# hku-mars/LiDAR_IMU_Init

Measured on AMD Instinct MI355X. Metric: ICP+ESKF scans/sec @100k pts/scan, higher is better.
Workload: dtype f64; 1 GPU; stream100k: 100000 pts/scan (time-sorted) vs 1000000-pt local map, max_iteration 5, LIO mode (12-col H), static map, voxel-grid leaf 0.05; scans resident in HBM, 8 distinct scans cycled, the state reset to the scan's propagated state every step; map_points=1000000, params=harness/launch/ouster (reference-format yaml + launch), parallelism=points sharded x1, transport=none, rccl_ranks=0

## Files before the change

### lidar_imu_init_amd/csrc/lii_capi.cpp

```cpp
#include "lii_context.h"

using namespace lii_impl;

namespace lii_impl {

thread_local std::string g_err;

static constexpr unsigned kProfEventFlags = hipEventDisableSystemFence;

void harvest_knn_events(lii_handle h) {
  const unsigned int due = h->prof.ev_it_due;
  h->prof.ev_it_due = 0u;
  for (int it = 0; it < 16; it++) {
    if (!((due >> it) & 1u)) continue;
    float kk = 0;
    if (hipEventElapsedTime(&kk, h->prof.ev_it[2 * it], h->prof.ev_it[2 * it + 1]) != hipSuccess) continue;
    h->prof.timings[7] += kk;
    h->prof.timings[5] += 1;
  }
}

int fail(lii_handle h, int code, const std::string& msg) {
  if (h) h->err = msg;
  g_err = msg;
  return code;
}
int kp_mark(lii_handle h, int kind, int it) {
  if (h->prof.prof_mode != 3) return LII_OK;
  if (h->prof.kp_n >= (int)h->prof.kp_ev.size()) {
    lii::Event e;
    if (e.create(kProfEventFlags) != hipSuccess) return fail(h, LII_ERR_HIP, "hipEventCreate (kernel profile)");
    h->prof.kp_ev.push_back(std::move(e));
    h->prof.kp_kind.push_back(0);
  }
  if (hipEventRecord(h->prof.kp_ev[size_t(h->prof.kp_n)], h->stream) != hipSuccess) return fail(h, LII_ERR_HIP, "hipEventRecord (kernel profile)");
  h->prof.kp_kind[size_t(h->prof.kp_n)] = kind * 64 + std::min(it, 63);
  h->prof.kp_n++;
  return LII_OK;
}
GridView grid_view(const lii_context* c) {
  GridView g;
  g.pts = c->d_pts;
  g.blocks = c->d_blocks;
  g.cells = c->d_cells;
  g.block_mask = c->block_mask;
  g.n_pts = c->map_dirty ? std::max(c->n_map, 1) : c->n_map;
  g.cs = c->cell_size;
  g.inv_cs = 1.0f / c->cell_size;
  g.max_d2 = c->cfg.max_match_dist2;
  g.win = (c->win_valid && !c->map_dirty) ? c->d_win : nullptr;
  g.wx0 = c->win_org[0]; g.wy0 = c->win_org[1]; g.wz0 = c->win_org[2];
  g.wnx = c->win_dim[0]; g.wny = c->win_dim[1]; g.wnz = c->win_dim[2];
  return g;
}
RegistrationBuffers reg_buffers(const lii_context* c) {
  RegistrationBuffers rb;
  rb.body = c->d_body;
  rb.world = c->d_world;
  rb.nbr = c->d_nbr;
  rb.nbr_count = c->d_nbr_count;
  rb.plane = c->d_plane;
  rb.selected = c->d_selected;
  rb.partials = c->d_partials;
  rb.partial_stride = c->partial_stride;
  rb.n = c->n_body;
  rb.n_dev = c->n_body_pending ? c->d_nbody : nullptr;
  rb.cap = c->cfg.max_scan_points;
  rb.flag_count = c->d_flags;
  rb.flag_list = reinterpret_cast<float4*>(c->d_flags + 4);
  rb.shard_rank = c->net.rank;
  rb.shard_world = (c->net.n_ranks > 1 && c->net.library_partition && !c->body_partitioned) ? c->net.n_ranks : 1;
  if (c->solo_share < -1 && c->net.n_ranks <= 1) { rb.shard_world = -c->solo_share; rb.shard_rank = 0; }
  return rb;
}
PoseArg pose_of(const lii_state& s) {
  PoseArg p;
  std::memcpy(p.R, s.rot_end, 72);
  std::memcpy(p.p, s.pos_end, 24);
  std::memcpy(p.RLI, s.offset_R_L_I, 72);
  std::memcpy(p.TLI, s.offset_T_L_I, 24);
  return p;
}
bool fuse_filter(lii_handle h, float leaf) {
  if (!(leaf > 0.f) || h->voxel_sort || h->no_fuse) return false;
  if (h->vh.part_world > 1) return true;
  return h->vh_mode == 1 && (h->vh_pinned || leaf == h->vh_leaf);
}
int resolve_n_body(lii_handle h) {
  if (!h->n_body_pending) return LII_OK;
  HIPCHK(h, hipMemcpyAsync(h->h_small + 2048, h->d_nbody, 2 * sizeof(int), hipMemcpyDeviceToHost, h->stream));
  HIPCHK(h, hipStreamSynchronize(h->stream));
  int v[2];
  std::memcpy(v, h->h_small + 2048, sizeof(v));
  h->n_body = v[0];
  h->last_filtered = v[1];
  h->n_body_pending = false;
  return LII_OK;
}

int pcl_order(lii_handle h, const int** perm) {
  *perm = nullptr;
  if (!h->body_reordered) return LII_OK;
  int rc = resolve_n_body(h);
  if (rc != LII_OK) return rc;
  if (!h->pcl_perm_valid) {
    const int n = h->n_body;
    std::vector<unsigned int> keys(size_t(std::max(n, 1)));
    if (n > 0) {
      HIPCHK(h, hipMemcpyAsync(h->h_stage, h->d_vpcl_out, sizeof(unsigned int) * size_t(n), hipMemcpyDeviceToHost, h->stream));
      HIPCHK(h, hipStreamSynchronize(h->stream));
      std::memcpy(keys.data(), h->h_stage, sizeof(unsigned int) * size_t(n));
    }
    h->pcl_perm.resize(size_t(n));
    for (int i = 0; i < n; i++) h->pcl_perm[size_t(i)] = i;
    std::sort(h->pcl_perm.begin(), h->pcl_perm.end(), [&](int a, int b) { return keys[size_t(a)] < keys[size_t(b)]; });
    h->pcl_perm_valid = true;
  }
  *perm = h->pcl_perm.data();
  return LII_OK;
}

void extent_discard(lii_handle h) {
  if (h->extent_valid) h->extent_sel ^= 1;
  h->extent_valid = false;
  h->scan_pending = nullptr;
  h->scan_pending_n = 0;
}
bool gate_move(lii::GateState* st, unsigned long long seq, unsigned long long to) {
  unsigned long long expect = (seq << 2) | lii::kGateArmed;
  return __atomic_compare_exchange_n(&st->word, &expect, (seq << 2) | to, false, __ATOMIC_ACQ_REL, __ATOMIC_ACQUIRE);
}
void prearm_cancel(lii_handle h) {
  if (!h || !h->pre.armed) return;
  h->pre.armed = false;
  if (gate_move(h->pre.state, h->pre.seq, lii::kGateCancel)) h->pre.n_cancelled++;
  else h->pre.n_expired++;
}
void intensity_detach(lii_handle h) {
  h->inten.have = false;
  h->inten.body_have = false;
}
int intensity_buffers(lii_handle h) {
  const size_t cap = size_t(h->cfg.max_scan_points);
  if (!h->inten.d_scan) HIPCHK(h, h->inten.d_scan.alloc(cap));
  if (!h->inten.d_body) HIPCHK(h, h->inten.d_body.alloc(cap));
  return LII_OK;
}
int scan_materialize(lii_handle h) {
  if (!h->scan_pending) return LII_OK;
  const float4* src = h->scan_pending;
  const int n = h->scan_pending_n;
  const bool keep = h->inten.have;
  const int rc = lii_scan_set_device(h, src, n);
  if (rc == LII_OK) h->inten.have = keep;
  return rc;
}
int scan_sort_into(lii_handle h, const float4* src, int n) {
  if (n <= 0) return LII_OK;
  lii_context::ScanSort& b = h->ssort;
  if (!b.d_temp) {
    const size_t cap = size_t(h->cfg.max_scan_points);
    HIPCHK(h, b.d_key_a.grow(cap));
    HIPCHK(h, b.d_key_b.grow(cap));
    HIPCHK(h, b.d_idx_a.grow(cap));
    HIPCHK(h, b.d_idx_b.grow(cap));
    HIPCHK(h, b.d_out.grow(cap));
    HIPCHK(h, b.d_temp.alloc(sort_temp_bytes(h->cfg.max_scan_points)));
  }
  hipStream_t s = h->stream;
  const bool in_place = src == h->d_scan.get();
  if (n == 1) {
    if (!in_place) HIPCHK(h, hipMemcpyAsync(h->d_scan, src, sizeof(float4), hipMemcpyDeviceToDevice, s));
    return LII_OK;
  }
  const bool wi = h->inten.have;
  if (wi && !h->inten.d_sort_out) HIPCHK(h, h->inten.d_sort_out.alloc(size_t(h->cfg.max_scan_points)));
  launch_sort_keys(src, n, b.d_key_a, b.d_idx_a, s);
  sort_pairs_u32(b.d_temp, b.d_temp.size(), b.d_key_a, b.d_key_b, b.d_idx_a, b.d_idx_b, n, s);
  launch_sort_gather(src, b.d_idx_b, n, in_place ? b.d_out.get() : h->d_scan.get(), s, wi ? h->inten.d_scan.get() : nullptr, wi ? h->inten.d_sort_out.get() : nullptr);
  HIPCHK(h, hipGetLastError());
  if (in_place) std::swap(h->d_scan, b.d_out);
  if (wi) std::swap(h->inten.d_scan, h->inten.d_sort_out);
  return LII_OK;
}
unsigned long long* extent_of_scan(lii_handle h) {
  unsigned long long* ext = h->d_extent + 2 * h->extent_sel;
  if (!h->extent_valid) {
    launch_time_extent(h->d_scan, h->n_scan, ext, h->d_extent + 2 * (h->extent_sel ^ 1), nullptr, h->h_ctrl, h->d_ctrl, h->ctrl_pending,
                       h->stream);
    h->ctrl_pending = 0;
  }
  h->extent_sel ^= 1;
  h->extent_valid = false;
  return ext;
}
lii::GatherView gather_view(lii_handle h) {
  lii::GatherView g;
  g.peers = h->net.mailbox.d_gather_peers;
  g.block_bytes = h->net.mailbox.gather_block;
  g.cap_points = h->net.mailbox.gather_cap;
  g.n_ranks = h->net.n_ranks;
  g.rank = h->net.rank;
  g.timeout_ticks = h->net.mailbox_timeout_ticks;
  return g;
}
MailboxView mailbox_view(lii_handle h) {
  MailboxView v;
  v.slots = h->net.mailbox.dev_slots;
  v.peers = h->net.mailbox.d_peers;
  v.seq = h->net.d_mb_seq;
  v.n_ranks = h->net.n_ranks;
  v.rank = h->net.rank;
  v.timeout_ticks = h->net.mailbox_timeout_ticks;
  v.handoff_ticks = h->test_sum_lost ? 20000000ll : 200000000ll;
  v.test_drop_sum = h->test_sum_lost ? 1 : 0;
  return v;
}

static void read_switches(lii_handle h) {
  if (const char* v = std::getenv("LII_DIAG")) h->diag = std::atoi(v) != 0;
  if (const char* v = std::getenv("LII_VOXEL_FILTER")) {
    h->voxel_sort = std::string(v) == "sort";
    if (std::string(v) == "hash") { h->vh_pinned = true; h->vh_mode = 1; }
  }
  if (const char* v = std::getenv("LII_KNN_PLAN")) h->knn_plan = std::atoi(v) != 0;
  if (const char* v = std::getenv("LII_WINDOW_KEEP")) h->win_keep = std::atoi(v) != 0;
  if (const char* v = std::getenv("LII_MAP_FUSE")) h->map_fuse = v[0] != '0';
  if (const char* v = std::getenv("LII_WIDE_COMPLETION")) h->wide_enabled = v[0] != '0';
  if (const char* v = std::getenv("LII_INGEST_SORT")) h->ingest_sort_always = v[0] == 'a';
  if (const char* v = std::getenv("LII_PREARM")) h->pre.enabled = std::atoi(v) != 0;
  if (const char* v = std::getenv("LII_PREARM_TIMEOUT_MS")) h->pre.timeout_ticks = std::max(1ll, (long long)(std::atof(v) * 1e5));
  if (const char* v = std::getenv("LII_MAILBOX_TIMEOUT_S")) {
    h->net.mailbox_timeout_ticks = (long long)(std::atof(v) * 1e8);
    if (const char* c = std::strchr(v, ',')) h->net.mailbox_wait_s = std::atof(c + 1);
  }
  if (const char* v = std::getenv("LII_TEST")) {
    const std::string t(v);
    for (size_t b = 0, e; b < t.size(); b = e + 1) {
      e = std::min(t.find(',', b), t.size());
      const std::string k = t.substr(b, e - b);
      if (k == "map_tight") h->map_tight = true;
      else if (k.compare(0, 11, "plan_force=") == 0) h->knn_plan_force = int(std::strtol(k.c_str() + 11, nullptr, 0) & 0x7FFFFFFF);
      else if (k == "host_solve") h->host_solve = true;
      else if (k == "sync_result") h->poll_result = false;
      else if (k == "pred_small") h->test_pred_small = true;
      else if (k == "fold_sort") h->fold_sorted = true;
      else if (k == "no_fuse") h->no_fuse = true;
      else if (k == "no_fast") h->no_fast_prologue = true;
      else if (k == "force_rebuild") h->test_force_rebuild = true;
      else if (k == "no_gather") h->no_gather = true;
      else if (k == "emit_late") h->test_emit_late = true;
      else if (k == "sum_lost") h->test_sum_lost = true;
      else if (k.compare(0, 11, "solo_share=") == 0) h->solo_share = int(std::strtol(k.c_str() + 11, nullptr, 0));
      else if (!k.empty()) std::fprintf(stderr, "[libliinit_hip] LII_TEST: unknown token '%s' ignored\n", k.c_str());
    }
  }
}

}

int lii_internal_fail(lii_context* h, int code, const std::string& msg) { return fail(h, code, msg); }
int lii_internal_scan_materialize(lii_context* h) { return scan_materialize(h); }
int lii_internal_scan_is_deferred(lii_context* h) { return h && h->scan_pending ? 1 : 0; }
int lii_internal_in_wait_hook(lii_context* h) { return h && h->in_wait_hook ? 1 : 0; }
void lii_internal_prearm_cancel(lii_context* h) { prearm_cancel(h); }
int lii_internal_scan_defer(lii_handle h, const void* dev_float4, int32_t n) {
  if (!h || (!dev_float4 && n > 0) || n < 0) return fail(h, LII_ERR_INVALID, "lii_frame_select: bad frame");
  if (n > h->cfg.max_scan_points) return fail(h, LII_ERR_CAPACITY, "lii_frame_select: frame larger than max_scan_points");
  extent_discard(h);
  intensity_detach(h);
  h->scan_buf_idle = false;
  h->bbox_rows = 0;
  h->scan_pending = n > 0 ? static_cast<const float4*>(dev_float4) : nullptr;
  h->scan_pending_n = n > 0 ? n : 0;
  h->n_scan = n;
  h->n_body = 0;
  h->n_body_pending = false;
  h->have_search = false;
  return LII_OK;
}

int lii_internal_intensity_refused(lii_context* h) { return h && (h->net.comm || h->net.n_ranks > 1 || h->host_solve) ? 1 : 0; }
int lii_internal_scan_intensity_adopt(lii_handle h, const float* dev_float, int32_t n) {
  if (!h) return LII_ERR_INVALID;
  intensity_detach(h);
  if (!dev_float || n <= 0 || n != h->n_scan) return LII_OK;
  { const int rc = intensity_buffers(h); if (rc != LII_OK) return rc; }
  HIPCHK(h, hipMemcpyAsync(h->inten.d_scan, dev_float, sizeof(float) * size_t(n), hipMemcpyDeviceToDevice, h->stream));
  h->inten.have = true;
  return LII_OK;
}

int lii_internal_li_init_on_device(lii_context* h) { return h && h->cal.li_init_device ? 1 : 0; }
hipStream_t lii_internal_stream(lii_context* h) { return h->stream; }
void** lii_internal_ingest_slot(lii_context* h) { return &h->ingest; }
void lii_internal_ingest_switches(lii_context* h, bool* diag, bool* sort_always) { *diag = h->diag; *sort_always = h->ingest_sort_always; }

extern "C" {

int lii_abi_version(void) { return LII_ABI_VERSION; }

const char* lii_strerror(int status) {
  switch (status) {
    case LII_OK: return "ok";
    case LII_ERR_INVALID: return "invalid argument";
    case LII_ERR_NO_DEVICE: return "no usable HIP device (libliinit_hip has no CPU fallback)";
    case LII_ERR_HIP: return "HIP runtime error";
    case LII_ERR_CAPACITY: return "capacity exceeded";
    case LII_ERR_STATE: return "call order violated";
    case LII_ERR_COMM: return "RCCL error";
    default: return "unknown status";
  }
}
const char* lii_last_error(lii_handle h) { return h ? h->err.c_str() : g_err.c_str(); }

int lii_device_count(int* count) {
  if (!count) return LII_ERR_INVALID;
  int n = 0;
  hipError_t e = hipGetDeviceCount(&n);
  if (e != hipSuccess) { *count = 0; return fail(nullptr, LII_ERR_NO_DEVICE, hipGetErrorString(e)); }
  *count = n;
  return LII_OK;
}

static int create_resources(lii_handle h) {
  const lii_config* cfg = &h->cfg;
  HIPCHK(h, hipSetDevice(h->device));
  hipDeviceProp_t prop;
  HIPCHK(h, hipGetDeviceProperties(&prop, h->device));
  if (std::string(prop.gcnArchName).find("gfx950") == std::string::npos)
    return fail(h, LII_ERR_NO_DEVICE, std::string("device is ") + prop.gcnArchName + ", kernels are built for gfx950 only");
  HIPCHK(h, h->stream.create(hipStreamNonBlocking));
  const size_t N = size_t(cfg->max_scan_points), M = size_t(cfg->max_map_points);
  const size_t NM = std::max(N, M);
  HIPCHK(h, h->d_map_unsorted.alloc(M));
  HIPCHK(h, h->d_map.alloc(M));
  h->pts_cap = (unsigned int)std::min<size_t>(3 * M + 65536, 0x7FFFFFF0u);
  HIPCHK(h, h->d_pts.alloc(size_t(h->pts_cap)));
  HIPCHK(h, h->d_work.alloc(std::min<size_t>(10 * NM + 4096, 0x7FFFFFF0u)));
  h->work_cap = (unsigned int)h->d_work.size();
  HIPCHK(h, h->d_ins_e.alloc(NM));
  HIPCHK(h, h->d_ins_e2.alloc(NM));
  HIPCHK(h, h->d_mapctr.alloc(kMapCtrWords + 8));
  HIPCHK(h, hipMemset(h->d_mapctr, 0, sizeof(int) * (kMapCtrWords + 8)));
  h->d_counts = h->d_mapctr + kMapCtrWords;
  HIPCHK(h, h->d_keys_a.alloc(M));
  HIPCHK(h, h->d_keys_b.alloc(M));
  HIPCHK(h, h->d_keys_c.alloc(M));
  HIPCHK(h, h->d_idx_a.alloc(M));
  HIPCHK(h, h->d_idx_b.alloc(M));
  HIPCHK(h, h->d_blocks.alloc(4096));
  h->block_mask = (unsigned int)h->d_blocks.size() - 1;
  const size_t cap_blocks = std::max<size_t>(4096, M / 64);
  HIPCHK(h, h->d_cells.alloc(cap_blocks * 512));
  HIPCHK(h, h->d_cell_cap.alloc(cap_blocks * 512));
  HIPCHK(h, h->d_tp.alloc(cap_blocks * 512));
  HIPCHK(h, h->d_cs_a.alloc(cap_blocks * 512));
  HIPCHK(h, h->d_cs_b.alloc(cap_blocks * 512));
  HIPCHK(h, h->d_block_key.alloc(cap_blocks));
  h->cells_cap_blocks = h->d_block_key.size();
  HIPCHK(h, hipMemset(h->d_cells, 0, sizeof(uint2) * h->cells_cap_blocks * 512));
  HIPCHK(h, hipMemset(h->d_cell_cap, 0, sizeof(unsigned int) * h->cells_cap_blocks * 512));
  HIPCHK(h, hipMemset(h->d_tp, 0, sizeof(unsigned int) * h->cells_cap_blocks * 512));
  HIPCHK(h, h->d_counter.alloc(4));
  HIPCHK(h, h->d_tomb.alloc((size_t(h->pts_cap) + 3) & ~size_t(3)));
  HIPCHK(h, hipMemset(h->d_tomb, 0, h->d_tomb.size()));
  HIPCHK(h, h->d_ins.alloc(M));
  HIPCHK(h, h->d_batch.alloc(M));
  HIPCHK(h, h->d_dropped.alloc(NM));
  h->drop_cap = (unsigned int)h->d_dropped.size();
  HIPCHK(h, h->d_ins_c.alloc(M));
  HIPCHK(h, h->d_u32_a.alloc(NM));
  HIPCHK(h, h->d_u32_b.alloc(NM));
  HIPCHK(h, hipMemset(h->d_u32_b, 0, sizeof(unsigned int) * NM));
  HIPCHK(h, h->d_u32_c.alloc(NM));
  {
    const size_t slots = add_hash_slots(int(N));
    HIPCHK(h, h->d_ah_key.alloc(slots)); HIPCHK(h, h->d_ah_best.alloc(slots)); HIPCHK(h, h->d_ah_slot.alloc(N));
    HIPCHK(h, hipMemset(h->d_ah_key, 0xFF, 8 * slots)); HIPCHK(h, hipMemset(h->d_ah_best, 0xFF, 8 * slots));
  }
  HIPCHK(h, h->d_list_add.alloc(N));
  HIPCHK(h, h->d_list_nodown.alloc(N));
  HIPCHK(h, h->n_map_pinned.alloc(16, hipHostMallocDefault));
  h->n_map_pinned[0] = 0;
  HIPCHK(h, h->d_sort_temp.alloc(sort_temp_bytes(int(std::max<size_t>(NM, h->cells_cap_blocks * 512)))));
  HIPCHK(h, h->d_scan.alloc(N));
  HIPCHK(h, h->d_body.alloc(N));
  HIPCHK(h, h->d_world.alloc(N));
  HIPCHK(h, h->d_nbr.alloc(N * kMatch));
  HIPCHK(h, h->d_nbr_count.alloc(N));
  HIPCHK(h, h->d_plane.alloc(N * 4));
  HIPCHK(h, h->d_selected.alloc(N));
  HIPCHK(h, h->d_nbody.alloc(4));
  {
    HIPCHK(h, h->d_ctrl_poses.alloc(kCtrlBytes + sizeof(lii_pose6d) * 1024 + 1024));
    h->d_ctrl = reinterpret_cast<IekfCtrl*>(h->d_ctrl_poses.get());
    h->d_poses = reinterpret_cast<double*>(h->d_ctrl_poses + kCtrlBytes);
  }
  HIPCHK(h, h->d_pose.alloc(1));
  HIPCHK(h, h->h_ctrl_poses.alloc(kCtrlBytes + sizeof(lii_pose6d) * 1024 + 1024, hipHostMallocDefault));
  h->h_ctrl = reinterpret_cast<IekfCtrl*>(h->h_ctrl_poses.get());
  h->h_poses = reinterpret_cast<lii_pose6d*>(h->h_ctrl_poses + kCtrlBytes);
  static_assert(sizeof(lii::GateState) == 8, "the state word's allocation is 64 bytes");
  HIPCHK(h, h->pre.state.alloc(8, hipHostMallocMapped));
  std::memset(h->pre.state, 0, 64);
  HIPCHK(h, h->pre.d_ring.alloc(size_t(lii::kGateRing) * lii::kGateLines * 8));
  HIPCHK(h, hipMemset(h->pre.d_ring, 0, sizeof(double) * size_t(lii::kGateRing) * lii::kGateLines * 8));
  HIPCHK(h, h->pre.d_flag.alloc(8));
  HIPCHK(h, hipMemset(h->pre.d_flag, 0, 64));
  {
    int large_bar = 0;
    if (hipDeviceGetAttribute(&large_bar, hipDeviceAttributeIsLargeBar, h->device) != hipSuccess) large_bar = 0;
    h->pre.enabled = h->pre.enabled && large_bar != 0;
  }
  HIPCHK(h, h->h_res.alloc(1, hipHostMallocMapped));
  std::memset(h->h_res, 0, sizeof(IekfResult));
  partition_refresh(h);
  HIPCHK(h, h->ev_poses.create(hipEventDisableTiming));
  HIPCHK(h, h->ev_stage.create(hipEventDisableTiming));
  HIPCHK(h, h->ev_mapflag.create(hipEventDisableTiming));
  HIPCHK(h, h->h_mapflag.alloc(64, hipHostMallocMapped));
  std::memset(h->h_mapflag, 0, 256);
  HIPCHK(h, h->ev_lists.create(hipEventDisableTiming));
  HIPCHK(h, hipMemset(h->d_counter, 0, 16));
  h->partial_stride = register_blocks(int(N)) + std::max(lii::kCompletionBlocks, lii::kCompletionBlocksPre) + 8;
  HIPCHK(h, h->d_flags.alloc(4 + 16 * lii::kListCap));
  HIPCHK(h, hipMemset(h->d_flags, 0, sizeof(int) * (4 + 16 * lii::kListCap)));
  HIPCHK(h, h->d_partials.alloc(size_t(h->partial_stride) * kNormalEq));
  HIPCHK(h, h->d_out91.alloc(256));
  HIPCHK(h, h->d_gran.alloc(256));
  HIPCHK(h, hipMemset(h->d_gran, 0, 8 * 256));
  HIPCHK(h, h->d_extent.alloc(4));
  HIPCHK(h, h->d_mm.alloc(16));
  HIPCHK(h, h->d_bbox_rows.alloc((N / 256 + 2) * 8));
  {
    const unsigned long long e0[4] = {~0ull, 0ull, ~0ull, 0ull};
    const unsigned int m0[16] = {~0u, ~0u, ~0u, 0, 0, 0, 0, 0, ~0u, ~0u, ~0u, 0, 0, 0, 0, 0};
    HIPCHK(h, hipMemcpy(h->d_extent, e0, sizeof(e0), hipMemcpyHostToDevice));
    HIPCHK(h, hipMemcpy(h->d_mm, m0, sizeof(m0), hipMemcpyHostToDevice));
  }
  HIPCHK(h, h->d_vkeys_a.alloc(N));
  HIPCHK(h, h->d_vkeys_b.alloc(N));
  HIPCHK(h, h->d_vidx_b.alloc(N));
  HIPCHK(h, h->d_vcomp.alloc(N));
  HIPCHK(h, h->d_vsplit.alloc(2048 + 4096));
  HIPCHK(h, h->d_vhist.alloc(voxel_sort_hist_elems((int)N)));
  HIPCHK(h, hipMemset(h->d_vhist, 0, sizeof(unsigned int) * voxel_sort_hist_elems((int)N)));
  HIPCHK(h, h->d_vbucket.alloc(N));
  HIPCHK(h, h->d_vpcl_in.alloc(N));
  HIPCHK(h, h->d_vpcl_out.alloc(N));
  {
    const size_t slots = voxel_hash_slots((int)N);
    HIPCHK(h, h->vh_slots.alloc(64 * slots));
    h->vh.slots = h->vh_slots;
    launch_voxel_hash_clear(h->vh, slots, h->stream);
    HIPCHK(h, h->vh_slot_of.alloc(N)); HIPCHK(h, h->vh_next.alloc(N));
    HIPCHK(h, h->vh_counts.alloc(N / 256 + 8)); HIPCHK(h, hipMemset(h->vh_counts, 0, 8 * (N / 256 + 8)));
    HIPCHK(h, h->vh_crowded.alloc(4));
    HIPCHK(h, hipMemset(h->vh_crowded, 0, 16));
    h->vh.slot_of = h->vh_slot_of; h->vh.next = h->vh_next; h->vh.counts = h->vh_counts; h->vh.crowded = h->vh_crowded;
    HIPCHK(h, h->h_vh_crowded.alloc(16, hipHostMallocDefault));
    *h->h_vh_crowded = 0;
    HIPCHK(h, h->ev_vh.create(hipEventDisableTiming));
  }
  HIPCHK(h, h->cal.d_cal_params.alloc(64));
  HIPCHK(h, h->cal.d_cal_out.alloc(128));
  HIPCHK(h, h->h_stage.alloc(NM * kMatch, hipHostMallocDefault));
  HIPCHK(h, h->h_small.alloc(32768, hipHostMallocDefault));
  for (int i = 0; i < 4; i++) HIPCHK(h, h->prof.ev[i].create(kProfEventFlags));
  for (int i = 0; i < 32; i++) HIPCHK(h, h->prof.ev_it[i].create(kProfEventFlags));
  launch_table_clear(h->d_blocks, (unsigned int)h->d_blocks.size(), h->stream);
  HIPCHK(h, hipStreamSynchronize(h->stream));
  return LII_OK;
}
static int fail_create(lii_handle h, int rc) {
  delete h;
  return rc;
}

int lii_create(const lii_config* cfg, lii_handle* out) {
  if (!cfg || !out || cfg->struct_size != (int32_t)sizeof(lii_config)) return fail(nullptr, LII_ERR_INVALID, "bad lii_config");
  if (cfg->max_scan_points <= 0 || cfg->max_map_points <= 0) return fail(nullptr, LII_ERR_INVALID, "capacities must be > 0");
  int ndev = 0;
  if (hipGetDeviceCount(&ndev) != hipSuccess || ndev <= 0)
    return fail(nullptr, LII_ERR_NO_DEVICE, "no HIP device visible; libliinit_hip has no CPU fallback");
  if (cfg->device < 0 || cfg->device >= ndev) return fail(nullptr, LII_ERR_INVALID, "device ordinal out of range");
  lii_handle h = new lii_context;
  h->cfg = *cfg;
  if (h->cfg.max_match_dist2 <= 0) h->cfg.max_match_dist2 = 5.0f;
  if (h->cfg.plane_threshold <= 0) h->cfg.plane_threshold = 0.1;
  if (h->cfg.laser_point_cov_inv <= 0) h->cfg.laser_point_cov_inv = 1000.0;
  if (h->cfg.map_downsample_size <= 0) h->cfg.map_downsample_size = 0.2f;
  h->cell_size = cfg->map_cell_size > 0 ? cfg->map_cell_size : 3.0f * h->cfg.map_downsample_size;
  h->cell_size = std::max(h->cell_size, std::sqrt(h->cfg.max_match_dist2) / 8.0f * 1.001f);
  read_switches(h);
  h->ds = h->cfg.map_downsample_size;
  h->device = cfg->device;
  const int rc = create_resources(h);
  if (rc != LII_OK) return fail_create(h, rc);
  *out = h;
  return LII_OK;
}

int lii_destroy(lii_handle h) {
  lii_internal_prearm_cancel(h);
  if (!h) return LII_OK;
  (void)hipSetDevice(h->device);
  if (h->net.comm) ncclCommDestroy(h->net.comm);
  if (h->copy_stream) (void)hipStreamSynchronize(h->copy_stream);
  if (h->map_stream) (void)hipStreamSynchronize(h->map_stream);
  if (h->stream) (void)hipStreamSynchronize(h->stream);
#ifdef LII_FALLBACK_TRACE
  {
    unsigned long long t[32] = {};
    lii::fb_trace_read(t);
    for (int kind = 0; kind < 2; kind++) {
      const unsigned long long* q = t + 8 * kind;
      if (q[0] == 0) continue;
      const double n = double(q[0]);
      std::fprintf(stderr, "[libliinit_hip completion trace] %s: %llu queries, us per query: head -> inner list %.2f, cell entries -> list %.2f, candidates %.2f, selection %.2f, "
                   "winners stored %.2f; chunks listed %.1f, cells of the cube %.0f\n", kind == 0 ? "balls of more than 256 cells" : "balls of up to 256 cells", q[0],
                   0.01 * q[1] / n, 0.01 * q[2] / n, 0.01 * q[3] / n, 0.01 * q[4] / n, 0.01 * q[5] / n, double(q[6]) / n, double(q[7]) / n);
    }
    if (t[0] > 0)
      std::fprintf(stderr, "[libliinit_hip completion trace] of 'cell entries -> list' (window rows only), us per query: until the block probes are in %.2f, waiting for the row loads %.2f, "
                   "list trips %.2f\n", 0.01 * t[24] / double(t[0]), 0.01 * t[25] / double(t[0]), 0.01 * t[26] / double(t[0]));
    if (t[16] > 0)
      std::fprintf(stderr, "[libliinit_hip completion trace] completion workgroups with work: %llu (%.2f queries each), us: head %.2f, completions %.2f, fit + sums %.2f\n", t[16],
                   double(t[20]) / double(t[16]), 0.01 * t[17] / double(t[16]), 0.01 * t[18] / double(t[16]), 0.01 * t[19] / double(t[16]));
  }
#endif
#ifdef LII_GAP_TRACE
  if (h->d_gran) {
    unsigned long long g[4] = {0, 0, 0, 0};
    if (hipMemcpy(g, h->d_gran + 200, sizeof(g), hipMemcpyDeviceToHost) == hipSuccess && g[2] > 0)
      std::fprintf(stderr, "[libliinit_hip gap trace] device idle between the stopping solve of a scan and the first kernel of the next: %.2f us mean over %llu "
                   "back-to-back scans (%llu gaps of 50 us or more left out)\n", 0.01 * double(g[1]) / double(g[2]), g[2], g[3]);
  }
#endif
  if (h->diag) std::fprintf(stderr, "[libliinit_hip] pre-armed prologues: %lld used, %lld cancelled, %lld expired\n", h->pre.n_used, h->pre.n_cancelled, h->pre.n_expired);
// ... 178 lines not shown
  if (!h->poses_preloaded) {
    if (h->staging_busy) { HIPCHK(h, hipStreamSynchronize(h->stream)); h->staging_busy = false; }
    HIPCHK(h, hipEventSynchronize(h->ev_poses));
    std::memcpy(h->h_poses, poses, sizeof(lii_pose6d) * size_t(n_poses));
    HIPCHK(h, hipMemcpyAsync(h->d_poses, h->h_poses, sizeof(lii_pose6d) * size_t(n_poses), hipMemcpyHostToDevice, h->stream));
    HIPCHK(h, hipEventRecord(h->ev_poses, h->stream));
  }
  h->poses_preloaded = false;
  UndistArgH u;
  std::memcpy(u.endR, end_R, 72);
  std::memcpy(u.endp, end_p, 24);
  std::memcpy(u.RLI, R_LI, 72);
  std::memcpy(u.TLI, T_LI, 24);
  unsigned long long* ext = extent_of_scan(h);
  h->vh_inserted = fuse_filter(h, h->fuse_leaf);
  if (h->vh_inserted) h->vh_inserted_leaf = h->fuse_leaf;
  DeskewPlan dp = {};
  dp.in = dp.out = h->d_scan; dp.n = h->n_scan; dp.sorted = 0; dp.extent = ext; dp.bbox_rows = h->d_bbox_rows;
  dp.leaf = h->fuse_leaf; dp.vh = h->vh_inserted ? &h->vh : nullptr;
  launch_deskew_imu(dp, nullptr, h->d_poses, n_poses, u, h->stream);
  h->bbox_rows = (h->n_scan + 255) / 256;
  HIPCHK(h, hipGetLastError());
  return LII_OK;
}
int lii_undistort_cv(lii_handle h, const double omega[3], const double vel[3], const double end_R[9]) {
  if (h) h->scan_buf_idle = false;
  lii_internal_prearm_cancel(h);
  if (!h || !omega || !vel || !end_R) return fail(h, LII_ERR_INVALID, "lii_undistort_cv: bad arguments");
  { const int rcm = scan_materialize(h); if (rcm != LII_OK) return rcm; }
  if (h->n_scan <= 0) return LII_OK;
  CvArgH a;
  std::memcpy(a.omega, omega, 24);
  std::memcpy(a.vel, vel, 24);
  std::memcpy(a.endR, end_R, 72);
  unsigned long long* ext = extent_of_scan(h);
  h->vh_inserted = fuse_filter(h, h->fuse_leaf);
  if (h->vh_inserted) h->vh_inserted_leaf = h->fuse_leaf;
  DeskewPlan dp = {};
  dp.in = dp.out = h->d_scan; dp.n = h->n_scan; dp.sorted = 0; dp.extent = ext; dp.bbox_rows = h->d_bbox_rows;
  dp.leaf = h->fuse_leaf; dp.vh = h->vh_inserted ? &h->vh : nullptr;
  launch_deskew_cv(dp, a, h->stream);
  h->bbox_rows = (h->n_scan + 255) / 256;
  HIPCHK(h, hipGetLastError());
  return LII_OK;
}
int lii_downsample_skip(lii_handle h, int32_t* n_down) {
  if (h) h->scan_buf_idle = false;
  lii_internal_prearm_cancel(h);
  if (!h) return LII_ERR_INVALID;
  { const int rcm = scan_materialize(h); if (rcm != LII_OK) return rcm; }
  if (h->prof.kp_active) { const int r = kp_mark(h, LII_KP_VOXEL); if (r != LII_OK) return r; }
  if (h->n_scan > 0)
    HIPCHK(h, hipMemcpyAsync(h->d_body, h->d_scan, sizeof(float4) * size_t(h->n_scan), hipMemcpyDeviceToDevice, h->stream));
  if (h->inten.have && h->n_scan > 0)
    HIPCHK(h, hipMemcpyAsync(h->inten.d_body, h->inten.d_scan, sizeof(float) * size_t(h->n_scan), hipMemcpyDeviceToDevice, h->stream));
  h->inten.body_have = h->inten.have;
  h->n_body = h->n_scan;
  h->n_body_pending = false;
  h->have_search = false;
  h->body_reordered = false;
  h->body_partitioned = false;
  if (n_down) *n_down = h->n_body;
  return LII_OK;
}
int lii_downsample(lii_handle h, float leaf, int32_t* n_down, int32_t* filtered) {
  if (h) h->scan_buf_idle = false;
  lii_internal_prearm_cancel(h);
  if (!h || !(leaf > 0)) return fail(h, LII_ERR_INVALID, "lii_downsample: bad arguments");
  { const int rcm = scan_materialize(h); if (rcm != LII_OK) return rcm; }
  h->have_search = false;
  h->n_body_pending = false;
  const int n = h->n_scan;
  if (h->inten.have && lii_internal_intensity_refused(h)) intensity_detach(h);
  const float* const inten = h->inten.have ? h->inten.d_scan.get() : nullptr;
  float* const inten_out = h->inten.have ? h->inten.d_body.get() : nullptr;
  h->inten.body_have = h->inten.have;
  if (n <= 0) {
    h->n_body = 0;
    if (n_down) *n_down = 0;
    if (filtered) *filtered = 1;
    return LII_OK;
  }
  hipStream_t s = h->stream;
  if (h->prof.kp_active) { const int r = kp_mark(h, LII_KP_VOXEL); if (r != LII_OK) return r; }
  unsigned int* mm = h->d_mm + 8 * h->mm_sel;
  if (h->bbox_rows == 0) {
    h->mm_sel ^= 1;
    launch_voxel_minmax(h->d_scan, n, mm, h->d_mm + 8 * h->mm_sel, s);
  }
  h->vh_calls++;
  if (h->vh_flag_pending && h->vh_calls >= h->vh_due) {
    HIPCHK(h, hipEventSynchronize(h->ev_vh));
    h->vh_flag_pending = false;
    if (h->vh_mode == 0 && *h->h_vh_crowded <= 32u) h->vh_mode = 1;
    else if (h->vh_mode == 1 && *h->h_vh_crowded > 64u) h->vh_mode = 0;
  }
  int hash_stages = 3;
  const bool inserted = h->vh_inserted;
  h->vh_inserted = false;
  if (inserted && leaf != h->vh_inserted_leaf) return fail(h, LII_ERR_STATE, "lii_downsample: the de-skew prepared the voxel filter for another leaf size");
  if (inserted) hash_stages = 4;
  if (!inserted && !h->vh_pinned && !h->voxel_sort && leaf != h->vh_leaf) {
    h->vh_leaf = leaf;
    h->vh_flag_pending = false;
    HIPCHK(h, hipMemsetAsync(h->vh.crowded, 0, sizeof(unsigned int), s));
    launch_voxel_hash(h->vh, h->d_scan, n, mm, h->d_bbox_rows, h->bbox_rows, leaf, h->d_body, h->d_nbody, h->d_nbody + 1, h->d_vpcl_out, 1, 0u, s);
    HIPCHK(h, hipMemcpyAsync(h->h_vh_crowded, h->vh.crowded, sizeof(unsigned int), hipMemcpyDeviceToHost, s));
    HIPCHK(h, hipMemsetAsync(h->vh.crowded, 0, sizeof(unsigned int), s));
    HIPCHK(h, hipStreamSynchronize(s));
    h->vh_mode = *h->h_vh_crowded > 32u ? 0 : 1;
    hash_stages = 2;
    if (h->vh_mode == 0)
      launch_voxel_hash_clear(h->vh, voxel_hash_slots(n), s);
  }
  const bool use_hash = inserted || (h->vh_mode == 1 && !h->voxel_sort);
  h->voxel_path_hash = use_hash;
  const bool by_voxel = inserted && h->vh.part_world > 1;
  if (use_hash) {
    if (++h->vh_epoch == 0u) h->vh_epoch = 1u;
    launch_voxel_hash(h->vh, h->d_scan, n, mm, h->d_bbox_rows, h->bbox_rows, leaf, h->d_body, h->d_nbody, h->d_nbody + 1, h->d_vpcl_out, hash_stages, h->vh_epoch, s, h->test_emit_late ? 1 : 0, inten, inten_out);
    if (!h->vh_pinned && !by_voxel && !h->vh_flag_pending && (++h->vh_watch & 15) == 0) {
      HIPCHK(h, hipMemcpyAsync(h->h_vh_crowded, h->vh.crowded, sizeof(unsigned int), hipMemcpyDeviceToHost, s));
      HIPCHK(h, hipMemsetAsync(h->vh.crowded, 0, sizeof(unsigned int), s));
      HIPCHK(h, hipEventRecord(h->ev_vh, s));
      h->vh_flag_pending = true;
      h->vh_due = h->vh_calls + 8;
    }
  } else {
    const VoxelSortPlan plan = voxel_sort_plan(n);
    launch_voxel_keys(h->d_scan, n, mm, h->d_bbox_rows, h->bbox_rows, leaf, h->d_vkeys_a, h->d_vpcl_in,
                      h->d_nbody + 1, plan.samples ? h->d_vsplit + 2048 : nullptr, plan.width, s);
    VoxelSortBuffers vb;
    vb.pcl_in = h->d_vpcl_in; vb.pcl_out = h->d_vpcl_out;
    vb.samples = h->d_vsplit + 2048;
    vb.keys_in = h->d_vkeys_a; vb.keys_out = h->d_vkeys_b; vb.idx_out = h->d_vidx_b;
    vb.comp = h->d_vcomp; vb.splitters = h->d_vsplit; vb.hist = h->d_vhist; vb.bucket_of = h->d_vbucket;
    vb.max_run = h->voxel_sort ? nullptr : h->vh.crowded;
    if (!h->voxel_sort) HIPCHK(h, hipMemsetAsync(h->vh.crowded, 0, sizeof(unsigned int), s));
    launch_voxel_sort_centroids(vb, h->d_scan, n, h->d_body, h->d_nbody, s, inten, inten_out);
    if (!h->voxel_sort && !h->vh_flag_pending && (++h->vh_watch & 15) == 0) {
      HIPCHK(h, hipMemcpyAsync(h->h_vh_crowded, h->vh.crowded, sizeof(unsigned int), hipMemcpyDeviceToHost, s));
      HIPCHK(h, hipMemsetAsync(h->vh.crowded, 0, sizeof(unsigned int), s));
      HIPCHK(h, hipEventRecord(h->ev_vh, s));
      h->vh_flag_pending = true;
      h->vh_due = h->vh_calls + 8;
    }
  }
  HIPCHK(h, hipGetLastError());
  h->n_body = by_voxel ? voxel_partition_bound(n, h->vh.part_world) : n;
  h->n_body_pending = true;
  h->body_partitioned = by_voxel;
  h->body_reordered = use_hash;
  h->pcl_perm_valid = false;
  if (n_down || filtered) {
    int rc = resolve_n_body(h);
    if (rc != LII_OK) return rc;
    if (n_down) *n_down = h->n_body;
    if (filtered) *filtered = h->last_filtered;
  }
  return LII_OK;
}
int lii_scan_download(lii_handle h, int32_t which, float* out_float4, int32_t capacity, int32_t* n) {
  lii_internal_prearm_cancel(h);
  if (!h || !n) return LII_ERR_INVALID;
  if (which == 0) { const int rcm = scan_materialize(h); if (rcm != LII_OK) return rcm; }
  const float4* src = which == 0 ? h->d_scan : (which == 1 ? h->d_body : h->d_world);
  if (which != 0) { int rc0 = resolve_n_body(h); if (rc0 != LII_OK) return rc0; }
  int cnt = which == 0 ? h->n_scan : h->n_body;
  *n = cnt;
  if (!out_float4) return LII_OK;
  if (capacity < cnt) return fail(h, LII_ERR_CAPACITY, "lii_scan_download: capacity too small");
  if (cnt > 0) {
    const int* perm = nullptr;
    if (which != 0) { int rc1 = pcl_order(h, &perm); if (rc1 != LII_OK) return rc1; }
    HIPCHK(h, hipMemcpyAsync(h->h_stage, src, sizeof(float4) * size_t(cnt), hipMemcpyDeviceToHost, h->stream));
    HIPCHK(h, hipStreamSynchronize(h->stream));
    if (!perm) std::memcpy(out_float4, h->h_stage, sizeof(float4) * size_t(cnt));
    else
      for (int r = 0; r < cnt; r++) std::memcpy(out_float4 + 4 * size_t(r), &h->h_stage[perm[r]], sizeof(float4));
  }
  return LII_OK;
}

static int intensity_attach_check(lii_handle h, const void* src, int32_t n, const char* who) {
  if (!h || (!src && n > 0) || n < 0) return fail(h, LII_ERR_INVALID, std::string(who) + ": bad arguments");
  if (lii_internal_intensity_refused(h)) return fail(h, LII_ERR_STATE, std::string(who) + ": single rank only for now (a communicator is attached, or LII_TEST=host_solve)");
  if (h->n_scan <= 0) return fail(h, LII_ERR_STATE, std::string(who) + ": no scan (lii_scan_upload / lii_scan_set_device / lii_scan_advance / lii_frame_select)");
  if (n != h->n_scan) return fail(h, LII_ERR_INVALID, std::string(who) + ": n is not the current scan's point count");
  return intensity_buffers(h);
}
int lii_scan_intensity_upload(lii_handle h, const void* points, int32_t n, int32_t stride_bytes, int32_t intensity_offset_bytes) {
  if (h) h->scan_buf_idle = false;
  lii_internal_prearm_cancel(h);
  if (h && (stride_bytes < 4 || intensity_offset_bytes < 0 || intensity_offset_bytes + 4 > stride_bytes))
    return fail(h, LII_ERR_INVALID, "lii_scan_intensity_upload: bad arguments");
  { const int rc = intensity_attach_check(h, points, n, "lii_scan_intensity_upload"); if (rc != LII_OK) return rc; }
  HIPCHK(h, hipEventSynchronize(h->ev_stage));
  float* st = reinterpret_cast<float*>(h->h_stage.get());
  const char* src = static_cast<const char*>(points);
  for (int i = 0; i < n; i++) std::memcpy(st + i, src + size_t(i) * stride_bytes + intensity_offset_bytes, 4);
  HIPCHK(h, hipMemcpyAsync(h->inten.d_scan, st, sizeof(float) * size_t(n), hipMemcpyHostToDevice, h->stream));
  HIPCHK(h, hipEventRecord(h->ev_stage, h->stream));
  h->inten.have = true;
// ... 82 lines not shown
```

### lidar_imu_init_amd/csrc/lii_capi_register.cpp

```cpp
#include "lii_context.h"
#include <cstddef>

#include "lii_hostmath.h"

using namespace lii_impl;

namespace {


int next_knn_epoch(lii_handle h) {
  h->knn_epoch = h->knn_epoch >= 0x3FFFFFFE ? 1 : h->knn_epoch + 1;
  return h->knn_epoch;
}
void launch_knn(lii_handle h, const GridView& g, const RegistrationBuffers& rb, const PoseArg* pose, int forced, int epoch,
                hipEvent_t ev_start = nullptr, hipEvent_t ev_stop = nullptr) {
  lii::launch_knn(g, rb, pose, h->d_ctrl, forced, h->d_ctrl->search_pose, h->stream, epoch, ev_start, ev_stop);
}


int iterate(lii_handle h, const lii_state* st, bool search, bool imu_en, double* out91) {
  if (h->n_body <= 0) return fail(h, LII_ERR_STATE, "no down-sampled scan (call lii_downsample / lii_downsample_skip)");
  int rc = commit_map(h);
  if (rc != LII_OK) return rc;
  if (!search && !h->have_search) return fail(h, LII_ERR_STATE, "non-search iteration before any search");
  GridView g = grid_view(h);
  RegistrationBuffers rb = reg_buffers(h);
  const bool prof = h->prof.profiling;
  if (prof) HIPCHK(h, hipEventRecord(h->prof.ev[0], h->stream));
  {
    PoseArg* stage = reinterpret_cast<PoseArg*>(h->h_small + 20000);
    *stage = pose_of(*st);
    HIPCHK(h, hipMemcpyAsync(h->d_pose, stage, sizeof(PoseArg), hipMemcpyHostToDevice, h->stream));
  }
  if (search) h->unfinished_known = false;
  const int epoch = search ? next_knn_epoch(h) : 0;
  if (search) launch_knn(h, g, rb, h->d_pose, 1, epoch);
  if (prof) HIPCHK(h, hipEventRecord(h->prof.ev[3], h->stream));
  launch_fit_reduce(g, rb, h->d_pose, h->d_ctrl, search ? 1 : 0, imu_en ? 1 : 0, h->cfg.plane_threshold,
                    h->cfg.laser_point_cov_inv, h->stream, epoch);
  if (prof) HIPCHK(h, hipEventRecord(h->prof.ev[1], h->stream));
  launch_reduce91(rb, h->d_out91, h->d_ctrl, 1, h->stream, epoch);
  if (prof) HIPCHK(h, hipEventRecord(h->prof.ev[2], h->stream));
  if (search) h->have_search = true;
  if (h->net.comm) {
    ncclResult_t r = ncclAllReduce(h->d_out91, h->d_out91, kNormalEq, ncclDouble, ncclSum, h->net.comm, h->stream);
    if (r != ncclSuccess) return fail(h, LII_ERR_COMM, std::string("ncclAllReduce: ") + ncclGetErrorString(r));
  } else if (h->net.mailbox.dev_slots) {
    launch_mailbox_allreduce(h->d_out91, mailbox_view(h), h->stream);
  }
  HIPCHK(h, hipMemcpyAsync(h->h_small, h->d_out91, sizeof(double) * kNormalEq, hipMemcpyDeviceToHost, h->stream));
  HIPCHK(h, hipStreamSynchronize(h->stream));
  std::memcpy(out91, h->h_small, sizeof(double) * kNormalEq);
  if (h->net.mailbox.dev_slots && out91[kNormalEq - 1] != out91[kNormalEq - 1])
    return fail(h, LII_ERR_COMM, "mailbox exchange timed out (a rank of the job did not reach this pass)");
  if (prof) {
    float a = 0, b = 0;
    HIPCHK(h, hipEventElapsedTime(&a, h->prof.ev[0], h->prof.ev[1]));
    HIPCHK(h, hipEventElapsedTime(&b, h->prof.ev[1], h->prof.ev[2]));
    if (search) {
      float k = 0;
      HIPCHK(h, hipEventElapsedTime(&k, h->prof.ev[0], h->prof.ev[3]));
      h->prof.timings[0] += a; h->prof.timings[5] += 1; h->prof.timings[7] += k;
    } else { h->prof.timings[1] += a; h->prof.timings[6] += 1; }
    h->prof.timings[2] += b;
  }
  return LII_OK;
}

void fill_ctrl(lii_handle h, const lii_state* state, const lii_state* state_prop, const lii_iekf_opts* opts) {
  IekfCtrl* hc = h->h_ctrl;
  std::memcpy(hc->st, state, sizeof(lii_state));
  std::memcpy(hc->prop, state_prop, sizeof(hc->prop));
  hc->max_it = opts->max_iterations;
  hc->imu_en = opts->imu_en;
  hc->it = 0; hc->search_next = 1; hc->stop = 0; hc->rematch_num = 0; hc->converged = 0; hc->searches = 0;
  hc->effect_num = 0; hc->singular = 0;
  h->update_seq = h->update_seq == 0x7FFFFFFF ? 1 : h->update_seq + 1;
  hc->seq = h->update_seq;
  unsigned int plan = 0xFFFFFFFFu;
  if (h->knn_plan && !h->net.comm && opts->max_iterations <= 16) {
    plan = (h->knn_plan_force >= 0 ? ((unsigned int)h->knn_plan_force | 0xFFFF0000u) : h->plan_next) | 0x00010001u;
  }
  hc->plan_mask = plan;
  h->plan_cur = plan;
}

int update_on_device(lii_handle h, lii_state* state, const lii_state* state_prop, const lii_iekf_opts* opts,
                     lii_iekf_report* report) {
  static_assert(sizeof(lii_state) == sizeof(double) * kStateDoubles, "lii_state layout");
  if (h->n_body <= 0) return fail(h, LII_ERR_STATE, "no down-sampled scan (call lii_downsample / lii_downsample_skip)");
  const auto t_map0 = std::chrono::steady_clock::now();
  int rc = commit_map(h);
  if (rc != LII_OK) return rc;
  if (h->diag) h->prof.host_map_us[0] += std::chrono::duration<double, std::micro>(std::chrono::steady_clock::now() - t_map0).count();
  hipStream_t s = h->stream;
  if (!h->map_stream && h->net.n_ranks <= 1) HIPCHK(h, h->map_stream.create(hipStreamNonBlocking));
  if (!h->ctrl_preloaded) {
    if (h->staging_busy) HIPCHK(h, hipStreamSynchronize(s));
    fill_ctrl(h, state, state_prop, opts);
    HIPCHK(h, hipMemcpyAsync(h->d_ctrl, h->h_ctrl, sizeof(IekfCtrl), hipMemcpyHostToDevice, s));
  }
  h->ctrl_preloaded = false;
  h->h_res->singular = 0;
  h->h_res->it = -1;
  if (h->lm.in_job) {
    rc = local_map_enqueue(h, h->d_ctrl->st + 9, nullptr, h->prof.kp_active);
    if (rc != LII_OK) return rc;
  }
  GridView g = grid_view(h);
  RegistrationBuffers rb = reg_buffers(h);
  const PoseArg* pose = reinterpret_cast<const PoseArg*>(h->d_ctrl);
  const bool prof = h->prof.profiling && h->prof.prof_mode != 3;
  if (prof) harvest_knn_events(h);
  const double* ne = h->net.comm ? h->d_out91 + 128 : h->d_out91;
  unsigned int plan = h->plan_cur;
  const unsigned int plan0 = plan;
  auto enqueue_pass = [&](int it) -> int {
    const bool knn = it >= 16 || ((plan >> it) & 1u);
    const int epoch = knn ? next_knn_epoch(h) : 0;
    if (knn) {
      if (h->prof.kp_active) { const int r = kp_mark(h, LII_KP_KNN, it); if (r != LII_OK) return r; }
      if (prof && it < 16) launch_knn(h, g, rb, pose, -1, epoch, h->prof.ev_it[2 * it], h->prof.ev_it[2 * it + 1]);
      else launch_knn(h, g, rb, pose, -1, epoch);
    }
    if (h->prof.kp_active) { const int r = kp_mark(h, LII_KP_FIT, it); if (r != LII_OK) return r; }
    if (knn && h->wide_listed && !h->net.comm && h->net.n_ranks <= 1) launch_complete_listed(g, rb, h->d_ctrl, -1, s, epoch);
    launch_fit_reduce(g, rb, pose, h->d_ctrl, -1, opts->imu_en ? 1 : 0, h->cfg.plane_threshold, h->cfg.laser_point_cov_inv, s, epoch);
    if (h->prof.kp_active) { const int r = kp_mark(h, LII_KP_SOLVE, it); if (r != LII_OK) return r; }
    if (!h->net.comm) {
      launch_reduce_solve(rb, h->d_gran, h->d_ctrl, h->h_res, mailbox_view(h), s, epoch);
      return LII_OK;
    }
    launch_reduce91(rb, h->d_out91, h->d_ctrl, -1, s, epoch);
    ncclResult_t r = ncclAllReduce(h->d_out91, h->d_out91 + 128, kNormalEq, ncclDouble, ncclSum, h->net.comm, s);
    if (r != ncclSuccess) return fail(h, LII_ERR_COMM, std::string("ncclAllReduce: ") + ncclGetErrorString(r));
    launch_iekf_solve(h->d_ctrl, ne, h->h_res, s);
    return LII_OK;
  };
  const auto t_loop0 = std::chrono::steady_clock::now();
  for (int it = 0; it < opts->max_iterations; it++) {
    if (it < 16 && !((plan >> (16 + it)) & 1u)) break;
    rc = enqueue_pass(it);
    if (rc != LII_OK) return rc;
  }
  auto wait_result = [&](bool first) -> int {
    const int parked_word = first ? (h->update_seq | kLoopParked) : h->update_seq;
    if (h->poll_result && !h->net.comm) {
      volatile int* done = &h->h_res->done;
      unsigned int spins = 0;
      while (*done != h->update_seq && *done != parked_word) {
        if ((++spins & 0x3FFF) == 0) {
          const hipError_t q = hipStreamQuery(s);
          if (q == hipSuccess) break;
          if (q != hipErrorNotReady) return fail(h, LII_ERR_HIP, std::string("hipStreamQuery: ") + hipGetErrorString(q));
        }
        __builtin_ia32_pause();
      }
      std::atomic_thread_fence(std::memory_order_acquire);
      if (*done != h->update_seq && *done != parked_word) HIPCHK(h, hipStreamSynchronize(s));
    } else {
      HIPCHK(h, hipStreamSynchronize(s));
    }
    return LII_OK;
  };
  if (h->diag) h->prof.host_loop_enq_us = std::chrono::duration<double, std::micro>(std::chrono::steady_clock::now() - t_loop0).count();
  if (h->prof.kp_active) { rc = kp_mark(h, LII_KP_KINDS); if (rc != LII_OK) return rc; }
  h->map_enqueued_early = false;
  if (h->map_after_update && !h->net.comm && !h->prof.profiling) {
    const auto t_me0 = std::chrono::steady_clock::now();
    h->map_enqueued_early = map_update_early(h) == 1;
    g = grid_view(h);
    if (h->diag) h->prof.host_map_us[1] += std::chrono::duration<double, std::micro>(std::chrono::steady_clock::now() - t_me0).count();
  }
  if (h->pub.on) { rc = publish_enqueue(h, h->d_ctrl, nullptr, true); if (rc != LII_OK) return rc; }
  if (h->pre.want_dev && !h->net.comm && h->net.n_ranks <= 1 && h->prof.prof_mode != 3 && !h->map_async && h->poll_result) {
    lii::GateState* gst = h->pre.state;
    h->pre.seq = (h->pre.seq + 1) & 0x003FFFFFFFFFFFFFull;
    __atomic_store_n(&gst->word, (h->pre.seq << 2) | lii::kGateArmed, __ATOMIC_RELEASE);
    h->pre.scan_dev = h->pre.want_dev; h->pre.n = h->pre.want_n; h->pre.leaf = h->pre.want_leaf; h->pre.late = h->pre.want_late;
    h->pre.fuse = fuse_filter(h, h->pre.leaf);
    DeskewPlan dp = {};
    dp.in = static_cast<const float4*>(h->pre.scan_dev);
    dp.out = h->pre.late ? const_cast<float4*>(dp.in) : h->d_scan;
    dp.n = h->pre.n; dp.sorted = 1; dp.extent = nullptr; dp.bbox_rows = h->d_bbox_rows;
    dp.leaf = h->pre.leaf; dp.vh = h->pre.fuse ? &h->vh : nullptr;
    dp.ctrl_src = h->h_ctrl; dp.ctrl_dst = h->d_ctrl; dp.ctrl_bytes = (sizeof(IekfCtrl) + 15) / 16 * 16;
#ifdef LII_GAP_TRACE
    dp.gap = h->d_gran;
#endif
    lii::DeskewGate gate = {gst, h->pre.d_ring + size_t(h->pre.seq % lii::kGateRing) * lii::kGateLines * 8, h->pre.d_flag, h->pre.seq, h->pre.timeout_ticks, h->pre.late ? 1 : 0};
    launch_deskew_imu_gated(dp, gate, s);
    h->pre.armed = hipGetLastError() == hipSuccess;
    if (!h->pre.armed) __atomic_store_n(&gst->word, (h->pre.seq << 2) | lii::kGateCancel, __ATOMIC_RELEASE);
  }
  h->pre.want_dev = nullptr;
  if (h->wait_hook) {
    void (*hook)(void*) = h->wait_hook;
    h->wait_hook = nullptr;
    h->in_wait_hook = true;
    hook(h->wait_hook_arg);
    h->in_wait_hook = false;
  }
  rc = wait_result(true);
// ... 330 lines not shown
        const unsigned long long tagw = (h->pre.seq << 2) | lii::kGateGo;
        std::memcpy(&tag, &tagw, 8);
        for (int l = 0; l < n_lines; l++)
          for (int c = 0; c < 7; c++) rec[8 * l + c] = pay[7 * l + c];
        __builtin_ia32_sfence();
        for (int l = 1; l < n_lines; l++) rec[8 * l + 7] = tag;
        __builtin_ia32_sfence();
        {
          const unsigned long long tag0 = tagw | ((unsigned long long)K << 56);
          double t0d;
          std::memcpy(&t0d, &tag0, 8);
          rec[7] = t0d;
        }
        __builtin_ia32_sfence();
      } else {
        use_pre = false;
        h->pre.n_expired++;
      }
    }
    DeskewPlan dp = {};
    dp.in = adopt ? static_cast<const float4*>(src_dev) : h->d_scan;
    dp.out = h->d_scan; dp.n = n_next; dp.sorted = 1; dp.extent = nullptr; dp.bbox_rows = h->d_bbox_rows;
    dp.leaf = fuse_leaf; dp.vh = h->vh_inserted ? &h->vh : nullptr;
    dp.ctrl_src = h->h_ctrl; dp.ctrl_dst = h->d_ctrl; dp.ctrl_bytes = (sizeof(IekfCtrl) + 15) / 16 * 16;
#ifdef LII_GAP_TRACE
    dp.gap = h->d_gran;
#endif
    if (use_pre) {
    } else if (job->undistort == 1) {
      UndistArgH u;
      std::memcpy(u.endR, state->rot_end, 72);
      std::memcpy(u.endp, state->pos_end, 24);
      std::memcpy(u.RLI, state->offset_R_L_I, 72);
      std::memcpy(u.TLI, state->offset_T_L_I, 24);
      launch_deskew_imu(dp, reinterpret_cast<const double*>(job->imu_poses), nullptr, job->n_imu_poses, u, h->stream);
    } else {
      CvArgH a;
      std::memcpy(a.omega, state->bias_g, 24);
      std::memcpy(a.vel, state->vel_end, 24);
      std::memcpy(a.endR, state->rot_end, 72);
      launch_deskew_cv(dp, a, h->stream);
    }
    h->bbox_rows = (n_next + 255) / 256;
    const hipError_t e_launch = hipGetLastError();
    if (e_launch != hipSuccess) { h->vh_inserted = false; h->ctrl_preloaded = false; rc = fail(h, LII_ERR_HIP, std::string("de-skew launch: ") + hipGetErrorString(e_launch)); }
  } else {
  if (job->undistort == 1 && !h->host_solve && job->imu_poses && job->n_imu_poses >= 2 && job->n_imu_poses <= 1024 && n_next > 0) {
    if (h->staging_busy) HIPCHK(h, hipStreamSynchronize(h->stream));
    HIPCHK(h, hipEventSynchronize(h->ev_poses));
    h->staging_busy = true;
    fill_ctrl(h, state, state_prop, &job->opts);
    std::memcpy(h->h_poses, job->imu_poses, sizeof(lii_pose6d) * size_t(job->n_imu_poses));
    const size_t bytes = kCtrlBytes + sizeof(lii_pose6d) * size_t(job->n_imu_poses);
    if (adopt || !h->extent_valid) {
      h->ctrl_pending = (bytes + 15) / 16 * 16;
    } else {
      HIPCHK(h, hipMemcpyAsync(h->d_ctrl, h->h_ctrl, (bytes + 1023) / 1024 * 1024, hipMemcpyHostToDevice, h->stream));
    }
    h->poses_preloaded = h->ctrl_preloaded = true;
  }
  if (adopt) {
    const bool keep = h->inten.have;
    rc = lii_scan_set_device(h, src_dev, src_n);
    if (rc == LII_OK) h->inten.have = keep;
    if (rc != LII_OK) { h->ctrl_pending = 0; h->poses_preloaded = h->ctrl_preloaded = false; return rc; }
  }
  if (job->undistort == 1) {
    h->fuse_leaf = job->leaf > 0 ? job->leaf : 0.f;
    rc = lii_undistort_imu(h, job->imu_poses, job->n_imu_poses, state->rot_end, state->pos_end, state->offset_R_L_I,
                           state->offset_T_L_I);
    h->fuse_leaf = 0.f;
    if (rc != LII_OK) h->vh_inserted = false;
  } else if (job->undistort == 2) {
    h->fuse_leaf = job->leaf > 0 ? job->leaf : 0.f;
    rc = lii_undistort_cv(h, state->bias_g, state->vel_end, state->rot_end);
    h->fuse_leaf = 0.f;
    if (rc != LII_OK) h->vh_inserted = false;
  }
  }
  if (h->ctrl_preloaded && h->ctrl_pending) {
    HIPCHK(h, hipMemcpyAsync(h->d_ctrl, h->h_ctrl, h->ctrl_pending, hipMemcpyHostToDevice, h->stream));
    h->ctrl_pending = 0;
  }
  if (rc == LII_OK) rc = job->leaf > 0 ? lii_downsample(h, job->leaf, nullptr, nullptr) : lii_downsample_skip(h, nullptr);
  const auto t_pre = std::chrono::steady_clock::now();
  const bool map_update = job->struct_size >= 56u && job->map_update == 1;
  h->map_after_update = map_update && !h->host_solve;
  h->map_enqueued_early = false;
  h->wait_hook = (rc == LII_OK && job->struct_size >= 88u) ? job->while_waiting : nullptr;
  h->wait_hook_arg = job->struct_size >= 88u ? job->while_waiting_arg : nullptr;
  h->lm.in_job = local_map && rc == LII_OK;
  if (rc == LII_OK) rc = lii_iekf_update(h, state, state_prop ? state_prop : state, &job->opts, report);
  if (h->lm.in_job) {
    if (rc == LII_OK) local_map_settle(h);
    else h->lm.counts_pending = true;
    h->lm.in_job = false;
  }
  if (h->wait_hook) {
    void (*hook)(void*) = h->wait_hook;
    h->wait_hook = nullptr;
    hook(h->wait_hook_arg);
  }
  h->map_after_update = false;
  if (rc == LII_OK && map_update && !h->map_enqueued_early) rc = lii_map_incremental(h, state, nullptr, nullptr);
  h->map_enqueued_early = false;
  h->poses_preloaded = h->ctrl_preloaded = false;
  h->prof.kp_active = false;
  if (h->diag) {
    const auto t_end = std::chrono::steady_clock::now();
    h->prof.host_us[0] += std::chrono::duration<double, std::micro>(t_first - t_entry).count();
    h->prof.host_us[1] += std::chrono::duration<double, std::micro>(t_pre - t_entry).count();
    h->prof.host_us[2] += h->prof.host_loop_enq_us;
    h->prof.host_us[3] += std::chrono::duration<double, std::micro>(t_end - t_entry).count();
    h->prof.host_us[4] += 1;
    h->prof.host_last_return = t_end;
  }
  if (rc == LII_OK && feed && feed->prop_out) std::memcpy(feed->prop_out, h->imu.h_out.get(), sizeof(lii_state));
  if (rc == LII_OK && cv && cv->prop_out) std::memcpy(cv->prop_out, h->imu.h_out.get(), sizeof(lii_state));
  return rc;
}

extern "C" {

int lii_last_solve_info(lii_handle h, int32_t* pivoted_passes) {
  if (!h || !pivoted_passes) return LII_ERR_INVALID;
  *pivoted_passes = h->last_pivoted_passes;
  return LII_OK;
}

int lii_last_unfinished_queries(lii_handle h, int32_t* n_last) {
  lii_internal_prearm_cancel(h);
  if (!h || !n_last) return LII_ERR_INVALID;
  if (h->unfinished_known) { *n_last = h->h_res->unfinished; return LII_OK; }
  int c[2] = {0, 0};
  HIPCHK(h, hipStreamSynchronize(h->stream));
  HIPCHK(h, hipMemcpy(c, h->d_flags, sizeof(c), hipMemcpyDeviceToHost));
  *n_last = c[h->knn_epoch & 1];
  return LII_OK;
}

int lii_iekf_iterate(lii_handle h, const lii_state* state, int32_t search, int32_t imu_en, double out91[91]) {
  lii_internal_prearm_cancel(h);
  if (!h || !state || !out91) return fail(h, LII_ERR_INVALID, "lii_iekf_iterate: bad arguments");
  return iterate(h, state, search != 0, imu_en != 0, out91);
}

int lii_iekf_update(lii_handle h, lii_state* state, const lii_state* state_prop, const lii_iekf_opts* opts,
                    lii_iekf_report* report) {
  lii_internal_prearm_cancel(h);
  if (!h || !state || !state_prop || !opts || opts->max_iterations < 1) return fail(h, LII_ERR_INVALID, "lii_iekf_update: bad arguments");
  const int max_it = opts->max_iterations;
  auto t_begin = std::chrono::steady_clock::now();
  if (!h->host_solve) {
    int rc = update_on_device(h, state, state_prop, opts, report);
    h->prof.timings[4] = std::chrono::duration<double, std::milli>(std::chrono::steady_clock::now() - t_begin).count();
    return rc;
  }
  double host_ms = 0;
  std::vector<double> Pinv(kDim * kDim), A(kDim * kDim), K1(kDim * kDim), KH(kDim * 12), G(kDim * kDim);
  if (!mat_inverse(state->cov, kDim, Pinv.data())) return fail(h, LII_ERR_INVALID, "state covariance is singular");
  int rematch_num = 0;
  bool search = true, stop = false, converged = false;
  int it = 0, searches = 0;
  double ne[kNormalEq];
  for (it = 0; it < max_it; it++) {
    int rc = iterate(h, state, search, opts->imu_en != 0, ne);
    if (rc != LII_OK) return rc;
    if (search) searches++;
    auto t0 = std::chrono::steady_clock::now();
    A = Pinv;
    double HTH[12][12];
    int t = 0;
    for (int i = 0; i < 12; i++)
      for (int j = i; j < 12; j++) { HTH[i][j] = ne[t]; HTH[j][i] = ne[t]; t++; }
    for (int i = 0; i < 12; i++)
// ... 93 lines not shown
```

### lidar_imu_init_amd/csrc/lii_context.h

```cpp
#pragma once
#include <hip/hip_runtime_api.h>
#include <rccl/rccl.h>

#include <algorithm>
#include <atomic>
#include <chrono>
#include <cmath>
#include <cstdio>
#include <cstdlib>
#include <cstring>
#include <string>
#include <vector>

#include "../../include/liinit_hip.h"
#include "lii_launch.h"
#include "lii_owned.h"

using lii::BlockEntry; using lii::IekfCtrl; using lii::IekfResult; using lii::PoseArg; using lii::VoxelHashBuffers; using lii::MailboxHost;
using lii::DevBuf; using lii::PinnedBuf;
constexpr size_t kCtrlBytes = (sizeof(lii::IekfCtrl) + 255) / 256 * 256;

struct lii_context {
  lii_config cfg{};
  int device = 0;
// ... 72 lines not shown
  const float4* scan_pending = nullptr;
  int scan_pending_n = 0;
  DevBuf<float4> d_scan_next;
  PinnedBuf<float4> h_stage_next;
  lii::Event ev_next;
  lii::Event ev_scan_free;
  int n_scan_next = -1;
  const void* pin_cache_ptr[8] = {};
  bool pin_cache_direct[8] = {};
  int pin_cache_at = 0;
  bool scan_buf_idle = false;
  struct ScanSort {
    DevBuf<unsigned int> d_key_a, d_key_b, d_idx_a, d_idx_b;
    DevBuf<float4> d_out;
    DevBuf<unsigned char> d_temp;
  } ssort;
  struct Intensity {
    DevBuf<float> d_scan;
    DevBuf<float> d_sort_out;
    DevBuf<float> d_body;
    bool have = false;
    bool body_have = false;
  } inten;
  DevBuf<float4> d_body;
  DevBuf<float4> d_world;
  DevBuf<float4> d_nbr;
  DevBuf<int> d_nbr_count;
  DevBuf<double> d_plane;
  DevBuf<unsigned char> d_selected;
  DevBuf<unsigned char> d_ctrl_poses;
  IekfCtrl* d_ctrl = nullptr;
  DevBuf<PoseArg> d_pose;
  PinnedBuf<unsigned char> h_ctrl_poses;
  IekfCtrl* h_ctrl = nullptr;
  PinnedBuf<IekfResult> h_res;
  lii_pose6d* h_poses = nullptr;
  int update_seq = 0;
  bool poll_result = true;
  bool poses_preloaded = false, ctrl_preloaded = false;
  lii::Event ev_poses;
  lii::Event ev_stage;
  bool host_solve = false;
  DevBuf<double> d_partials;
  DevBuf<double> d_out91;
  DevBuf<unsigned long long> d_gran;
  DevBuf<unsigned long long> d_extent;
  DevBuf<unsigned int> d_mm;
  int extent_sel = 0, mm_sel = 0;
  bool knn_plan = true;
  bool test_pred_small = false;
  bool test_force_rebuild = false;
  int solo_share = 0;
  bool no_gather = false;
  bool no_fast_prologue = false;
  bool no_fuse = false;
  bool test_sum_lost = false;
  bool test_emit_late = false;
  int plan_passes_prev = 32;
  int knn_plan_force = -1;
  unsigned int plan_next = 0xFFFFFFFFu, plan_cur = 0xFFFFFFFFu;
  long long map_repeats = 0;
  long long plan_parked = 0;
  bool staging_busy = false;
  size_t ctrl_pending = 0;
  bool extent_valid = false;
  DevBuf<unsigned int> d_bbox_rows;
  int bbox_rows = 0;
  DevBuf<unsigned long long> d_vkeys_a, d_vkeys_b;
  DevBuf<unsigned int> d_vidx_b;
  DevBuf<unsigned long long> d_vcomp, d_vsplit;
  DevBuf<unsigned int> d_vhist;
  DevBuf<unsigned short> d_vbucket;
  DevBuf<unsigned int> d_vpcl_in, d_vpcl_out;
  VoxelHashBuffers vh = {};
  DevBuf<unsigned char> vh_slots;
  DevBuf<unsigned int> vh_slot_of, vh_next, vh_crowded;
  DevBuf<unsigned long long> vh_counts;
  unsigned int vh_epoch = 0;
  bool voxel_sort = false;
  bool vh_pinned = false;
  float fuse_leaf = 0.f;
  float vh_inserted_leaf = 0.f;
  bool vh_inserted = false;
  int vh_mode = 1;
  float vh_leaf = -1.f;
  unsigned int vh_watch = 0;
  unsigned long long vh_calls = 0, vh_due = 0;
  bool voxel_path_hash = false;
  PinnedBuf<unsigned int> h_vh_crowded;
  lii::Event ev_vh;
  bool vh_flag_pending = false;
  bool body_partitioned = false;
  bool body_reordered = false;
  std::vector<int> pcl_perm;
  bool pcl_perm_valid = false;
  double* d_poses = nullptr;
  int n_scan = 0, n_body = 0;
  bool n_body_pending = false;
  int last_filtered = 1;
  DevBuf<int> d_nbody;
  bool body_is_scan = false;
  bool have_search = false;
  DevBuf<int> d_flags;
  int knn_epoch = 0;
  int last_pivoted_passes = 0;
  bool map_async = false;
  int bound_add = 0, bound_nodown = 0;
  int list_hist[8][2] = {};
  int list_hist_n = 0;
  int pred_add = -1, pred_nodown = -1;
  bool map_after_update = false;
  bool map_enqueued_early = false;
  bool lists_predicted = false;
  lii::Event ev_lists;
  PinnedBuf<int> h_mapflag;
  lii::Event ev_mapflag;
  unsigned int decide_epoch = 0;
  int map_seq = 0;
  bool map_flag_pending = false;
  bool diag = false;

  struct Prearm {
    PinnedBuf<lii::GateState> state;
    DevBuf<double> d_ring;
    DevBuf<unsigned long long> d_flag;
    unsigned long long seq = 0;
    bool enabled = true;
    bool armed = false;
    const void* scan_dev = nullptr;
    int n = 0;
    float leaf = 0.f;
    bool fuse = false;
    bool late = false;
    bool want_late = false;
    const void* want_dev = nullptr;
    int want_n = 0;
    float want_leaf = 0.f;
    long long timeout_ticks = 200000000ll;
    long long n_used = 0, n_cancelled = 0, n_expired = 0;
  } pre;

  PinnedBuf<float4> h_stage;
  PinnedBuf<double> h_small;

  struct CalibState {
    DevBuf<double> d_cal_imu, d_cal_lidar, d_cal_params, d_cal_out;
    int n_cal = 0;

    bool li_init_device = false;
  } cal;
  struct ImuState {
    lii_imu_noise noise{};
    bool have_noise = false, have_carry = false;
    DevBuf<double> d_buf;
    int carry_sel = 0;
    PinnedBuf<double> h_in;
    PinnedBuf<double> h_out;
    double* d_carry(int sel) const { return d_buf.get() + lii::kImuCarryDoubles * sel; }
    int* d_n_poses() const { return reinterpret_cast<int*>(d_buf.get() + 2 * lii::kImuCarryDoubles); }
    double* d_state() const { return d_buf.get() + 2 * lii::kImuCarryDoubles + 8; }
  } imu;
  struct Publish {
    static constexpr int kClouds = 4;
    bool on = false;
    int clouds = 0, to_host = 0, save_capacity = 0;
    DevBuf<float4> d_cloud[kClouds][2];
// ... 15 lines not shown
    DevBuf<float4> d_save;
    DevBuf<int> d_save_ctl;
    int save_par = 0;
    int cur = 0, have = -1;
    int n_scan_at[2] = {0, 0};
    int clouds_at[2] = {0, 0};
    int kp_idx = -1;
  } pub;
  struct LocalMap {
    bool set = false;
    bool enabled = false;
    float det_range = 0.f;
    lii::LocalMapParams P{};
    DevBuf<lii::LocalMapState> d_state;
    PinnedBuf<lii::LocalMapState> h_state;
    int cur = 0;
    int seq = 0;
    bool in_job = false;
    bool counts_pending = false;
  } lm;
  struct Removed {
    bool set = false;
    bool on = false;
    int cap = 0;
    DevBuf<float4> d_buf;
    DevBuf<unsigned long long> d_ctr;
    long long collected_base = 0, lost_base = 0;
  } rm;
  void* ingest = nullptr;
  bool ingest_sort_always = false;

  struct CommState {
    ncclComm_t comm = nullptr;
    MailboxHost mailbox;
    DevBuf<unsigned long long> d_mb_seq;
    DevBuf<unsigned int> d_gather_ticket;
    DevBuf<unsigned char> d_gx;
    size_t gx_block = 0; int gx_ranks = 0;
    unsigned long long gather_seq = 0;
    long long mailbox_timeout_ticks = 3000000000ll;
    double mailbox_wait_s = 20.0;
    int n_ranks = 1, rank = 0;
    std::string comm_why;
    bool library_partition = true;
    bool voxel_partition = false;
  } net;

  struct ProfState {
    bool kp_active = false;
    int prof_mode = 0;
    std::vector<lii::Event> kp_ev;
    std::vector<int> kp_kind;
    int kp_n = 0;
    lii_kernel_profile kprof{};
    bool profiling = false;
    lii::Event ev[4];
    lii::Event ev_it[32];
    unsigned int ev_it_due = 0u;
    double timings[8] = {0, 0, 0, 0, 0, 0, 0, 0};
    double host_map_us[2] = {0, 0};
    double host_us[6] = {0, 0, 0, 0, 0, 0};
    std::chrono::steady_clock::time_point host_last_return;
    double host_loop_enq_us = 0;
  } prof;
};


namespace lii_impl {
using namespace lii;

int fail(lii_handle h, int code, const std::string& msg);
inline unsigned int next_pow2(unsigned int v) {
  unsigned int p = 1;
  while (p < v) p <<= 1;
  return p;
}
int kp_mark(lii_handle h, int kind, int it = 0);
void harvest_knn_events(lii_handle h);
GridView grid_view(const lii_context* c);
RegistrationBuffers reg_buffers(const lii_context* c);
PoseArg pose_of(const lii_state& s);
int resolve_n_body(lii_handle h);
bool fuse_filter(lii_handle h, float leaf);
int pcl_order(lii_handle h, const int** perm);
void extent_discard(lii_handle h);
int scan_sort_into(lii_handle h, const float4* src, int n);
void intensity_detach(lii_handle h);
int intensity_buffers(lii_handle h);
int scan_materialize(lii_handle h);
bool gate_move(lii::GateState* st, unsigned long long seq, unsigned long long to);
void prearm_cancel(lii_handle h);
unsigned long long* extent_of_scan(lii_handle h);
MailboxView mailbox_view(lii_handle h);
lii::GatherView gather_view(lii_handle h);
int build_index(lii_handle h, int n, int extra_blocks = 0);
void note_list_sizes(lii_handle h, int n_add, int n_nodown);
int map_join(lii_handle h);
constexpr int kMapFlagSeqAt = 40;
int map_update_early(lii_handle h);
int commit_map(lii_handle h);
int map_counters(lii_handle h, bool already_synced = false);
lii::RemovedSink removed_sink(lii_handle h);
lii::WinKeep win_keep_view(lii_handle h);
int local_map_enqueue(lii_handle h, const double* pos_dev, const double* pos, bool mark);
void local_map_settle(lii_handle h);
int map_gather(lii_handle h, int* n_out);
int map_rebuild(lii_handle h, int extra_blocks);
int map_apply(lii_handle h, const float4* list, int n_list, bool downsample, const float4* extra, int n_extra, bool beside = false,
              const int* n_list_dev = nullptr, const int* n_extra_dev = nullptr, bool count_events = true, bool prefilled = false);
struct ImuFeed {
  const lii_imu_sample* imu;
  int n_imu;
  double pcl_beg_time;
  lii_state* prop_out;
};
struct CvFeed {
  double dt;
  const double* cov_gyr_scale;
  const double* cov_acc_scale;
  lii_state* prop_out;
};
int scan_register_job(lii_handle h, const lii_scan_job* job, lii_state* state, const lii_state* state_prop, lii_iekf_report* report, const ImuFeed* feed,
                      const CvFeed* cv = nullptr);
int imu_buffers(lii_handle h);
int publish_enqueue(lii_handle h, const IekfCtrl* guard, const PoseArg* ps, bool first);
void publish_finish(lii_handle h);
void comm_drop(lii_handle h);
void partition_refresh(lii_handle h);
int lists_exchange_rccl(lii_handle h, hipStream_t s);
}
```

### lidar_imu_init_amd/csrc/lii_knn.hip

```cpp
#include <hip/hip_runtime.h>
#include <hip/hip_ext.h>
#include <math.h>
#include <stdint.h>
#include <utility>

#include "lii_search.h"
#include "lii_launch.h"

namespace lii {


template <int NC>
__device__ __forceinline__ void lookup_cells_batched(const GridView& g, const uint4* __restrict__ tab, const int (&ix)[NC],
                                                     const int (&iy)[NC], const int (&iz)[NC], const bool (&want)[NC],
                                                     uint2 (&out)[NC]) {
  const int bb = kCellBias >> kCoarseShift;
  if (g.win) {
    unsigned int wi[NC];
    bool in[NC];
#pragma unroll
    for (int t = 0; t < NC; t++) {
      const unsigned int ux = (unsigned)(ix[t] - g.wx0), uy = (unsigned)(iy[t] - g.wy0), uz = (unsigned)(iz[t] - g.wz0);
      in[t] = ux < (unsigned)g.wnx && uy < (unsigned)g.wny && uz < (unsigned)g.wnz;
      wi[t] = in[t] ? (uz * (unsigned)g.wny + uy) * (unsigned)g.wnx + ux : 0u;
    }
#pragma unroll
    for (int t = 0; t < NC; t++) out[t] = (want[t] && in[t]) ? g.win[wi[t]] : make_uint2(0u, 0u);
    return;
  }
  unsigned long long bk[NC];
  unsigned int sl[NC];
  uint4 e[NC];
#pragma unroll
  for (int t = 0; t < NC; t++) {
    const int bx = (ix[t] >> kCoarseShift) + bb, by = (iy[t] >> kCoarseShift) + bb, bz = (iz[t] >> kCoarseShift) + bb;
    bk[t] = pack_block(bx, by, bz);
    sl[t] = hash_block(bx, by, bz) & g.block_mask;
  }
#pragma unroll
  for (int t = 0; t < NC; t++) e[t] = want[t] ? tab[sl[t]] : make_uint4(0xFFFFFFFFu, 0xFFFFFFFFu, 0u, 0u);
  unsigned int ci[NC];
  bool hit[NC];
#pragma unroll
  for (int t = 0; t < NC; t++) {
    unsigned long long ek = ((unsigned long long)e[t].y << 32) | e[t].x;
    while (want[t] && ek != bk[t] && ek != kEmptyKey) {
      sl[t] = (sl[t] + 1) & g.block_mask;
      e[t] = tab[sl[t]];
      ek = ((unsigned long long)e[t].y << 32) | e[t].x;
    }
    hit[t] = want[t] && ek == bk[t];
    ci[t] = e[t].z * (unsigned)kBlockCells + ((((unsigned)iz[t] & 7u) << 6) | (((unsigned)iy[t] & 7u) << 3) | ((unsigned)ix[t] & 7u));
  }
#pragma unroll
  for (int t = 0; t < NC; t++) out[t] = hit[t] ? g.cells[ci[t]] : make_uint2(0u, 0u);
}


__device__ __forceinline__ double pose_element(const PoseArg& ps, int t) {
  double v = 0;
#pragma unroll
  for (int e = 0; e < 9; e++) { v = t == e ? ps.R[e] : v; v = t == 12 + e ? ps.RLI[e] : v; }
#pragma unroll
  for (int e = 0; e < 3; e++) { v = t == 9 + e ? ps.p[e] : v; v = t == 21 + e ? ps.TLI[e] : v; }
  return v;
}

struct QueryCell {
  int cx, cy, cz, ox, oy, oz;
  float eps, g0, guard;
};
__device__ __forceinline__ QueryCell query_cell(const GridView& g, float wx, float wy, float wz) {
  QueryCell q;
  const float cs = g.cs;
  q.eps = 1e-6f * (fabsf(wx) + fabsf(wy) + fabsf(wz) + 8.f);
  q.cx = cell_of(wx, g.inv_cs); q.cy = cell_of(wy, g.inv_cs); q.cz = cell_of(wz, g.inv_cs);
  const float fx = fminf(fmaxf(wx - (float)q.cx * cs, 0.f), cs), fy = fminf(fmaxf(wy - (float)q.cy * cs, 0.f), cs),
              fz = fminf(fmaxf(wz - (float)q.cz * cs, 0.f), cs);
  q.ox = fx < 0.5f * cs ? -1 : 1; q.oy = fy < 0.5f * cs ? -1 : 1; q.oz = fz < 0.5f * cs ? -1 : 1;
  q.g0 = fminf(fminf(fmaxf(fx, cs - fx), fmaxf(fy, cs - fy)), fmaxf(fz, cs - fz)) - 2.f * q.eps;
  const float mfrac = fmaxf(fminf(fminf(fminf(fx, cs - fx), fminf(fy, cs - fy)), fminf(fz, cs - fz)), 0.f);
  q.guard = cs + mfrac - 2.f * q.eps;
  return q;
}

constexpr unsigned int kPkInf = 0xFFFFFFFFu;

struct Pk7 {
  unsigned int k0, k1, k2, k3, k4, k5, k6;
// ... 38 lines not shown
template <int LPQ>
__device__ __forceinline__ void pk_group_merge(Pk7& L) {
  if (LPQ >= 2) pk_merge<0xB1>(L);
  if (LPQ == 4) pk_merge<0x4E>(L);
}
template <int LPQ, int J>
__device__ __forceinline__ float group_bcast_f(float v) {
  if (LPQ == 4) return quad_perm_f<J * 0x55>(v);
  if (LPQ == 2) return quad_perm_f<J == 0 ? 0xA0 : 0xF5>(v);
  return v;
}
template <class F, int... I>
__device__ __forceinline__ void static_for_impl(F&& f, std::integer_sequence<int, I...>) {
  (f(std::integral_constant<int, I>{}), ...);
}
template <int N, class F>
__device__ __forceinline__ void static_for(F&& f) {
  static_for_impl(f, std::make_integer_sequence<int, N>{});
}
template <class T>
__device__ __forceinline__ T by_value(T x) { return x; }
template <int LPQ, int BASE, int N, class T>
__device__ __forceinline__ T pick_by_lane(const T (&arr)[N], int sub) {
  T v = by_value(arr[BASE < N ? BASE : N - 1]);
  static_for<LPQ - 1>([&](auto jc) {
    constexpr int j = decltype(jc)::value + 1;
    v = sub == j ? by_value(arr[BASE + j < N ? BASE + j : N - 1]) : v;
  });
  return v;
}

template <int LPQ>
struct CkGeom {
  static constexpr int kLaneShift = LPQ == 4 ? 2 : (LPQ == 2 ? 1 : 0);
  static constexpr int kChunkBits = 6;
  static constexpr int MAXCH = 1 << kChunkBits;
  static constexpr int kPosBits = kChunkBits + kLaneShift;
  static constexpr unsigned int kPosMask = (1u << kPosBits) - 1u;
  static constexpr int NR = 8 / LPQ;
  static constexpr int NW = (7 + LPQ - 1) / LPQ;
  static constexpr int MAXPASS = (19 + 2 * LPQ - 1) / (2 * LPQ);
};
template <int LPQ>
__device__ __forceinline__ void group_prefix(unsigned int v, int sub, unsigned int& before, unsigned int& total) {
  if (LPQ == 4) {
    const unsigned int v0 = quad_perm<0x00>(v), v1 = quad_perm<0x55>(v), v2 = quad_perm<0xAA>(v), v3 = quad_perm<0xFF>(v);
    before = sub == 0 ? 0u : (sub == 1 ? v0 : (sub == 2 ? v0 + v1 : v0 + v1 + v2));
    total = v0 + v1 + v2 + v3;
  } else if (LPQ == 2) {
    const unsigned int v0 = quad_perm<0xA0>(v), v1 = quad_perm<0xF5>(v);
    before = sub == 0 ? 0u : v0;
    total = v0 + v1;
  } else {
    before = 0u;
    total = v;
  }
}
template <int LPQ, int NC>
__device__ __forceinline__ void ck_write_chunks(unsigned int* __restrict__ tab, unsigned int at, const uint2 (&r)[NC]) {
#pragma unroll
  for (int t = 0; t < NC; t++) {
    for (unsigned int j = r[t].x; j < r[t].y; j += LPQ) tab[at++] = (j << 3) | min((unsigned)LPQ, r[t].y - j);
  }
}
template <int LPQ, int NB>
__device__ __forceinline__ void ck_scan(const float4* __restrict__ pts, const unsigned int* __restrict__ tab, unsigned int first, unsigned int end,
                                        int sub, float wx, float wy, float wz, Pk7& L) {
  using G = CkGeom<LPQ>;
  for (unsigned int base = first; base < end; base += NB) {
    unsigned int w[NB];
#pragma unroll
    for (int u = 0; u < NB; u++) w[u] = tab[base + u];
    F3 P[NB];
#pragma unroll
    for (int u = 0; u < NB; u++) P[u] = load_xyz(pts, (w[u] >> 3) + min((unsigned)sub, (w[u] & 7u) - 1u));
#pragma unroll
    for (int u = 0; u < NB; u++) {
      const float d = dist2_ref(wx, wy, wz, P[u].x, P[u].y, P[u].z);
      const unsigned int key = (__float_as_uint(d) & ~G::kPosMask) | (((base + u) << G::kLaneShift) | (unsigned)sub);
      pk_insert(L, (unsigned)sub < (w[u] & 7u) ? key : kPkInf);
    }
  }
}
template <int LPQ, int BS, int NB, int WPE>
__global__ __launch_bounds__(BS, WPE) void k_knn_ck(GridView g, RegistrationBuffers rb, const PoseArg* __restrict__ pose,
                                               const IekfCtrl* __restrict__ ctrl, int forced, int nb_real,
                                               double* __restrict__ search_pose_out, int epoch) {
  using G = CkGeom<LPQ>;
  constexpr int QPB = BS / LPQ;
  __shared__ unsigned int s_tab[QPB * (G::MAXCH + NB)];
  const int blk = xcd_remap(blockIdx.x, nb_real);
  const int sub = threadIdx.x & (LPQ - 1);
  const int ql = blk * QPB + (int)(threadIdx.x / LPQ);
  const bool early = rb.shard_world <= 1;
  float4 pb_early = make_float4(0.f, 0.f, 0.f, 0.f);
  if (early) pb_early = rb.body[min(max(ql, 0), rb.cap - 1)];
  const HeadScalars hs = load_head_scalars(pose, &ctrl->search_next, rb.n_dev ? rb.n_dev : &ctrl->max_it, &ctrl->max_it);
  const PoseArg& ps = hs.ps;
  const int c_search = hs.search_next, c_stop = hs.stop, n_mem = hs.n_mem;
  int lo, n_live;
  shard_range_n(rb, n_mem, lo, n_live);
  if (epoch > 0 && blockIdx.x == 0 && threadIdx.x == 0) rb.flag_count[(epoch + 1) & 1] = 0;
  if (forced < 0 && (c_stop || !c_search)) return;
  if (search_pose_out && blockIdx.x == 0 && threadIdx.x < 24) search_pose_out[threadIdx.x] = pose_element(ps, threadIdx.x);
  if (blk >= nb_real) return;
  if (blk * QPB + (int)((threadIdx.x & ~63u) / LPQ) >= n_live) return;
  const int qi = lo + ql;
  const bool live = ql < n_live;
  float wx = 0, wy = 0, wz = 0;
  if (live && sub == 0) body_to_world(ps, early ? pb_early : rb.body[qi], wx, wy, wz);
  wx = group_bcast_f<LPQ, 0>(wx); wy = group_bcast_f<LPQ, 0>(wy); wz = group_bcast_f<LPQ, 0>(wz);
  const bool active = live && g.n_pts > 0;
  const float INF = __builtin_inff();
  const uint4* __restrict__ tab_blocks = reinterpret_cast<const uint4*>(g.blocks);
  const float4* __restrict__ pts = g.pts;
  unsigned int* const tab = s_tab + (threadIdx.x / LPQ) * (G::MAXCH + NB);

  const QueryCell q = query_cell(g, wx, wy, wz);
  const float g0sq = q.g0 * q.g0, guardsq = q.guard * q.guard;
  unsigned int n_chunks;
  bool ovf;
  {
    uint2 r[G::NR];
    int jx[G::NR], jy[G::NR], jz[G::NR];
    bool want[G::NR];
#pragma unroll
    for (int t = 0; t < G::NR; t++) {
      const int c = sub * G::NR + t;
      jx[t] = q.cx + ((c & 1) ? q.ox : 0); jy[t] = q.cy + ((c & 2) ? q.oy : 0); jz[t] = q.cz + ((c & 4) ? q.oz : 0);
      want[t] = true;
    }
    lookup_cells_batched<G::NR>(g, tab_blocks, jx, jy, jz, want, r);
    unsigned int mine = 0u;
#pragma unroll
    for (int t = 0; t < G::NR; t++) {
      if (!active) r[t] = make_uint2(0u, 0u);
      mine += (r[t].y - r[t].x + (unsigned)LPQ - 1u) / (unsigned)LPQ;
    }
    unsigned int before;
    group_prefix<LPQ>(mine, sub, before, n_chunks);
    ovf = n_chunks > (unsigned)G::MAXCH;
    if (ovf) n_chunks = 0u;
    else ck_write_chunks<LPQ, G::NR>(tab, before, r);
    if (sub == 0) {
#pragma unroll
      for (int u = 0; u < NB - 1; u++) tab[n_chunks + u] = 0u;
    }
  }
  __builtin_amdgcn_fence(__ATOMIC_RELEASE, "wavefront");
  __builtin_amdgcn_wave_barrier();
  __builtin_amdgcn_fence(__ATOMIC_ACQUIRE, "wavefront");
  const bool fast = active && !ovf;
  Pk7 L;
  L.k0 = L.k1 = L.k2 = L.k3 = L.k4 = L.k5 = L.k6 = kPkInf;
  ck_scan<LPQ, NB>(pts, tab, 0u, n_chunks, sub, wx, wy, wz, L);
  pk_group_merge<LPQ>(L);

  {
    const float ub5 = L.k4 != kPkInf ? __uint_as_float(L.k4 | G::kPosMask) : INF;
    const float bound = fminf(ub5, g.max_d2);
    const bool need2 = fast && !(bound <= g0sq);
    if (__any(need2)) {
      float GX[3], GY[3], GZ[3];
      {
        const float nx = axis_gap(wx, q.cx + q.ox, g.cs, q.eps), fx = axis_gap(wx, q.cx - q.ox, g.cs, q.eps);
        const float ny = axis_gap(wy, q.cy + q.oy, g.cs, q.eps), fy = axis_gap(wy, q.cy - q.oy, g.cs, q.eps);
        const float nz = axis_gap(wz, q.cz + q.oz, g.cs, q.eps), fz = axis_gap(wz, q.cz - q.oz, g.cs, q.eps);
        GX[0] = 0.f; GX[1] = nx * nx; GX[2] = fx * fx;
        GY[0] = 0.f; GY[1] = ny * ny; GY[2] = fy * fy;
        GZ[0] = 0.f; GZ[1] = nz * nz; GZ[2] = fz * fz;
      }
      unsigned int m = 0u;
      static_for<27>([&](auto cc) {
        constexpr int c = decltype(cc)::value, sx = c % 3, sy = (c / 3) % 3, sz = c / 9;
        if constexpr (sx == 2 || sy == 2 || sz == 2) {
          const float d = GX[sx] + GY[sy] + GZ[sz];
          m |= d > bound ? 0u : (1u << c);
        }
      });
      m = need2 ? m : 0u;
      if (sub != 0) L.k0 = L.k1 = L.k2 = L.k3 = L.k4 = L.k5 = L.k6 = kPkInf;
      unsigned int t = m;
#pragma unroll
      for (int j = 0; j < LPQ - 1; j++) t = j < sub ? (t & (t - 1u)) : t;
      for (int pass = 0; pass < G::MAXPASS; pass++) {
        if (!__any(t != 0u)) break;
        const int c1 = t ? __ffs((int)t) - 1 : -1;
#pragma unroll
        for (int j = 0; j < LPQ; j++) t = t & (t - 1u);
        const int c2 = t ? __ffs((int)t) - 1 : -1;
#pragma unroll
        for (int j = 0; j < LPQ; j++) t = t & (t - 1u);
        uint2 r[2];
// ... 5 lines not shown
          jx[0] = q.cx + step(ca % 3, q.ox); jy[0] = q.cy + step((ca / 3) % 3, q.oy); jz[0] = q.cz + step(ca / 9, q.oz);
          jx[1] = q.cx + step(cb % 3, q.ox); jy[1] = q.cy + step((cb / 3) % 3, q.oy); jz[1] = q.cz + step(cb / 9, q.oz);
          lookup_cells_batched<2>(g, tab_blocks, jx, jy, jz, want, r);
        }
        if (c1 < 0) r[0] = make_uint2(0u, 0u);
        if (c2 < 0) r[1] = make_uint2(0u, 0u);
        const unsigned int mine = (r[0].y - r[0].x + (unsigned)LPQ - 1u) / (unsigned)LPQ + (r[1].y - r[1].x + (unsigned)LPQ - 1u) / (unsigned)LPQ;
        unsigned int before, add;
        group_prefix<LPQ>(mine, sub, before, add);
        const unsigned int from = n_chunks;
        if (from + add > (unsigned)G::MAXCH) {
          ovf = true;
          t = 0u;
          add = 0u;
        } else {
          ck_write_chunks<LPQ, 2>(tab, from + before, r);
        }
        n_chunks = from + add;
        if (sub == 0) {
#pragma unroll
          for (int u = 0; u < NB - 1; u++) tab[n_chunks + u] = 0u;
        }
        __builtin_amdgcn_fence(__ATOMIC_RELEASE, "wavefront");
        __builtin_amdgcn_wave_barrier();
        __builtin_amdgcn_fence(__ATOMIC_ACQUIRE, "wavefront");
        ck_scan<LPQ, NB>(pts, tab, from, n_chunks, sub, wx, wy, wz, L);
      }
      pk_group_merge<LPQ>(L);
    }
  }

  float e[7];
  F3 W[G::NW];
  float d7t;
  bool tie = false;
  {
    const unsigned int K[7] = {L.k0, L.k1, L.k2, L.k3, L.k4, L.k5, L.k6};
    float el[G::NW];
    static_for<G::NW>([&](auto ic) {
      constexpr int i = decltype(ic)::value;
      const unsigned int key = pick_by_lane<LPQ, LPQ * i>(K, sub);
      const unsigned int pos = key == kPkInf ? 0u : (key & G::kPosMask);
      W[i] = load_xyz(pts, (tab[pos >> G::kLaneShift] >> 3) + (pos & (unsigned)(LPQ - 1)));
    });
#pragma unroll
    for (int w = 0; w < 6; w++) tie = tie || ((K[w] ^ K[w + 1]) <= G::kPosMask && K[w + 1] != kPkInf);
    d7t = K[6] != kPkInf ? __uint_as_float(K[6] & ~G::kPosMask) : INF;
#pragma unroll
    for (int i = 0; i < G::NW; i++) el[i] = dist2_ref(wx, wy, wz, W[i].x, W[i].y, W[i].z);
    e[0] = group_bcast_f<LPQ, 0 % LPQ>(el[0 / LPQ]); e[1] = group_bcast_f<LPQ, 1 % LPQ>(el[1 / LPQ]);
    e[2] = group_bcast_f<LPQ, 2 % LPQ>(el[2 / LPQ]); e[3] = group_bcast_f<LPQ, 3 % LPQ>(el[3 / LPQ]);
    e[4] = group_bcast_f<LPQ, 4 % LPQ>(el[4 / LPQ]); e[5] = group_bcast_f<LPQ, 5 % LPQ>(el[5 / LPQ]);
    e[6] = group_bcast_f<LPQ, 6 % LPQ>(el[6 / LPQ]);
#pragma unroll
    for (int w = 0; w < 7; w++) e[w] = (K[w] != kPkInf && e[w] <= g.max_d2) ? e[w] : INF;
  }
  int rk[G::NW];
#pragma unroll
  for (int i = 0; i < G::NW; i++) rk[i] = sub + LPQ * i;
  float d5 = e[4];
  if (__any(tie)) {
    int rank[7];
#pragma unroll
    for (int w = 0; w < 7; w++) rank[w] = 0;
#pragma unroll
    for (int v = 0; v < 7; v++)
#pragma unroll
      for (int w = v + 1; w < 7; w++) {
        const bool swapped = e[v] > e[w];
        rank[w] += swapped ? 0 : 1;
        rank[v] += swapped ? 1 : 0;
      }
    d5 = INF;
#pragma unroll
    for (int w = 0; w < 7; w++) d5 = rank[w] == 4 ? e[w] : d5;
    static_for<G::NW>([&](auto ic) {
      constexpr int i = decltype(ic)::value;
      rk[i] = pick_by_lane<LPQ, LPQ * i>(rank, sub);
    });
  }
  const int found = e[4] < INF ? 5 : (e[3] < INF ? 4 : (e[2] < INF ? 3 : (e[1] < INF ? 2 : (e[0] < INF ? 1 : 0))));
  const bool amb = d7t < INF && !(d5 < d7t);
  const bool need = active && (ovf || amb || !(fminf(d5, g.max_d2) <= guardsq));
  if (live) {
    static_for<G::NW>([&](auto ic) {
      constexpr int i = decltype(ic)::value;
      const float ei = pick_by_lane<LPQ, LPQ * i>(e, sub);
      if (sub + LPQ * i < 7 && ei < INF && rk[i] < 5) rb.nbr[(size_t)rk[i] * rb.cap + qi] = make_float4(W[i].x, W[i].y, W[i].z, ei);
    });
    if (found < 5) {
#pragma unroll
      for (int r = 0; r < 5; r += LPQ)
        if (sub + r < 5 && sub + r >= found) rb.nbr[(size_t)(sub + r) * rb.cap + qi] = make_float4(0.f, 0.f, 0.f, INF);
    }
    if (sub == (LPQ > 1 ? 1 : 0)) {
      const int cflags = found | (need ? (kNeedy | ((ovf || amb) ? 0 : kCovered)) : 0);
      rb.nbr_count[qi] = cflags;
      if (need && epoch > 0) {
        const int at = atomicAdd(&rb.flag_count[epoch & 1], 1);
        if (at < kListCap) {
          float4* e = rb.flag_list + 2 * ((epoch & 1) * kListCap + at);
          e[0] = make_float4(wx, wy, wz, __int_as_float(qi));
          e[1] = make_float4(__int_as_float(cflags), 0.f, 0.f, 0.f);
        }
      }
    }
    if (sub == (LPQ == 4 ? 2 : 0)) rb.world[qi] = make_float4(wx, wy, wz, 0.f);
  }
}

static inline int nblk(int n, int b) { return (n + b - 1) / b; }
constexpr int kKnnBs = 128, kKnnNb = 6, kKnnWpe = 7;
void launch_knn(const GridView& g, const RegistrationBuffers& rb, const PoseArg* pose,
                const IekfCtrl* ctrl, int forced, double* search_pose_out, hipStream_t s, int epoch, hipEvent_t ev_start, hipEvent_t ev_stop) {
  int nq = nblk(shard_bound(rb), kKnnBs / 4);
  if (nq < 1) nq = 1;
  const int nq_pad = ((nq + 7) / 8) * 8;
  if (ev_start && ev_stop) {
    hipExtLaunchKernelGGL((k_knn_ck<4, kKnnBs, kKnnNb, kKnnWpe>), dim3(nq_pad), dim3(kKnnBs), 0, s, ev_start, ev_stop, 0u, g, rb, pose, ctrl, forced, nq,
                          search_pose_out, epoch);
    return;
  }
  hipLaunchKernelGGL((k_knn_ck<4, kKnnBs, kKnnNb, kKnnWpe>), dim3(nq_pad), dim3(kKnnBs), 0, s, g, rb, pose, ctrl, forced, nq, search_pose_out, epoch);
}
}
```

### lidar_imu_init_amd/csrc/lii_launch.h

```cpp
#pragma once
#include <hip/hip_runtime_api.h>
#include <stddef.h>

#include <string>

#include "lii_device.h"
#include "lii_fov.h"

struct lii_context;
int lii_internal_fail(lii_context* h, int code, const std::string& msg);
#define HIPCHK(h, call)                                                                                            \
  do {                                                                                                             \
    hipError_t e_ = (call);                                                                                        \
    if (e_ != hipSuccess) return lii_internal_fail(h, LII_ERR_HIP, std::string(#call) + ": " + hipGetErrorString(e_)); \
  } while (0)
int lii_internal_scan_defer(lii_context* h, const void* dev_float4, int32_t n);
int lii_internal_scan_materialize(lii_context* h);
int lii_internal_in_wait_hook(lii_context* h);
int lii_internal_scan_is_deferred(lii_context* h);
int lii_internal_intensity_refused(lii_context* h);
int lii_internal_scan_intensity_adopt(lii_context* h, const float* dev_float, int32_t n);
void lii_internal_prearm_cancel(lii_context* h);
hipStream_t lii_internal_stream(lii_context* h);
void** lii_internal_ingest_slot(lii_context* h);
void lii_internal_ingest_switches(lii_context* h, bool* diag, bool* sort_always);

namespace lii {
void ingest_destroy(void* slot);

struct UndistArgH { double endR[9], endp[3], RLI[9], TLI[3]; };
struct CvArgH { double omega[3], vel[3], endR[9]; };

void launch_map_keys(const float4* pts, int n, float inv_cs, unsigned long long* keys, unsigned int* idx, hipStream_t s);
void launch_map_gather(const float4* src, const unsigned int* idx, int n, float4* dst, hipStream_t s);
void launch_body_to_map(const float4* body, int n, const PoseArg& ps, float4* dst, hipStream_t s);
void launch_block_flags(const unsigned long long* keys, int n, unsigned int* flags, hipStream_t s);
void launch_table_clear(BlockEntry* blocks, unsigned int cap, hipStream_t s);
void launch_win_bbox(const BlockEntry* blocks, unsigned int cap, unsigned int* box, hipStream_t s);
void launch_win_fill(const BlockEntry* blocks, unsigned int cap, const uint2* cells, uint2* win, const int org[3], const int dim[3], hipStream_t s);
void launch_cells_fill(const unsigned long long* keys, const unsigned int* ranks, int n, BlockEntry* blocks,
                       unsigned int block_mask, uint2* cells, unsigned long long* key_of_id, hipStream_t s);
void launch_map_nearest(const GridView& g, unsigned int n_entries, unsigned int pts_cap, const void* queries, int n, int stride_bytes, int k,
                        float max_d2, int r_max, float* pts_out, float* d2_out, int* count_out, hipStream_t s);
void launch_knn(const GridView& g, const RegistrationBuffers& rb, const PoseArg* pose,
                const IekfCtrl* ctrl, int forced, double* search_pose_out, hipStream_t s, int epoch,
                hipEvent_t ev_start = nullptr, hipEvent_t ev_stop = nullptr);
#ifdef LII_FALLBACK_TRACE
void fb_trace_read(unsigned long long out[32]);
#endif
void launch_knn_complete(const GridView& g, const RegistrationBuffers& rb, hipStream_t s);
void launch_complete_listed(const GridView& g, const RegistrationBuffers& rb, const IekfCtrl* ctrl, int forced, hipStream_t s, int epoch);
void launch_fit_reduce(const GridView& g, const RegistrationBuffers& rb, const PoseArg* pose,
                       const IekfCtrl* ctrl, int forced, int imu_en, double plane_thr, double rinv, hipStream_t s, int epoch);
void launch_reduce91(const RegistrationBuffers& rb, double* out91, const IekfCtrl* ctrl, int forced, hipStream_t s, int epoch);
void launch_reduce_solve(const RegistrationBuffers& rb, unsigned long long* gran, IekfCtrl* c, IekfResult* res, const MailboxView& mb,
                         hipStream_t s, int epoch);
void launch_mailbox_allreduce(double* out91, const MailboxView& mb, hipStream_t s);
struct MailboxHost {
  void* map = nullptr;
  size_t bytes = 0;
  double* dev_slots = nullptr;
  bool registered = false;
  char name[64] = {0};
  double* own = nullptr;
  double* peer_ptr[64] = {nullptr};
  double** d_peers = nullptr;
  int n_peers = 0;
  unsigned char** d_gather_peers = nullptr;
  size_t gather_block = 0;
  int gather_cap = 0;
};
size_t mailbox_segment_bytes(int n_ranks);
int mailbox_open(const uint8_t id[128], int n_ranks, int rank, double wait_s, bool want_hbm, int gather_points, MailboxHost* m, std::string* why);
void launch_lists_push(const GatherView& gv, const float4* src_add, const float4* src_nodown, const int* counts, unsigned int* ticket,
                       unsigned long long seq, hipStream_t s);
void launch_lists_collect(const GatherView& gv, unsigned long long seq, float4* dst_add, float4* dst_nodown, int* counts, int err_at, hipStream_t s);
void launch_lists_exchange(const GatherView& gv, const float4* src_add, const float4* src_nodown, int* counts, int err_at, unsigned int* ticket,
                           unsigned long long seq, float4* dst_add, float4* dst_nodown, hipStream_t s);
void mailbox_close(MailboxHost* m);
void launch_loop_resume(IekfCtrl* c, unsigned int plan_mask, hipStream_t s);
void launch_iekf_solve(IekfCtrl* c, const double* ne, IekfResult* res, hipStream_t s);
int register_blocks(int n);
void launch_time_extent(const float4* pts, int n, unsigned long long* extent, unsigned long long* extent_next, float4* copy_to,
                        const void* ctrl_src, void* ctrl_dst, size_t ctrl_bytes, hipStream_t s);
void launch_sort_keys(const float4* pts, int n, unsigned int* key, unsigned int* idx, hipStream_t s);
void launch_sort_gather(const float4* src, const unsigned int* idx, int n, float4* dst, hipStream_t s, const float* inten_src = nullptr, float* inten_dst = nullptr);
void launch_voxel_minmax(const float4* pts, int n, unsigned int* mm, unsigned int* mm_next, hipStream_t s);
void launch_voxel_keys(const float4* pts, int n, const unsigned int* mm, const unsigned int* bbox_rows, int n_rows, float leaf,
                       unsigned long long* keys, unsigned int* pcl_keys, int* filtered_dev,
                       unsigned long long* samples, int sample_width, hipStream_t s);
struct VoxelHashBuffers {
  void* slots;
  unsigned int *slot_of, *next;
  unsigned long long* counts;
  unsigned int* crowded;
  int part_world, part_rank;
  int* part_overflow;
};
size_t voxel_hash_slots(int max_n);
int voxel_partition_bound(int n, int world);
void launch_voxel_hash_clear(const VoxelHashBuffers& vh, size_t slots, hipStream_t s);
void launch_voxel_hash(const VoxelHashBuffers& vh, const float4* pts, int n, const unsigned int* mm, const unsigned int* bbox_rows,
                       int n_rows, float leaf, float4* out, int* n_out, int* filtered, unsigned int* pcl_out, int stages, unsigned int epoch,
                       hipStream_t s, int test_late = 0 ,
                       const float* inten = nullptr, float* inten_out = nullptr);
struct DeskewPlan {
  const float4* in;
  float4* out;
  int n;
  int sorted;
  const unsigned long long* extent;
  unsigned int* bbox_rows;
  float leaf;
  const VoxelHashBuffers* vh;
  const void* ctrl_src;
  void* ctrl_dst;
  size_t ctrl_bytes;
#ifdef LII_GAP_TRACE
  unsigned long long* gap;
#endif
};
void launch_deskew_imu(const DeskewPlan& p, const double* poses_host, const double* poses_dev, int K, const UndistArgH& u, hipStream_t s);
constexpr unsigned long long kGateArmed = 0ull, kGateGo = 1ull, kGateCancel = 2ull, kGateExpired = 3ull;
constexpr int kGateMaxPoses = 29;
constexpr int kGateLines = (25 + 22 * kGateMaxPoses + 6) / 7;
constexpr int kGateRing = 64;
struct GateState { unsigned long long word; };
struct DeskewGate {
  GateState* host;
  const double* rec;
  unsigned long long* dev_flag;
  unsigned long long seq;
  long long timeout_ticks;
  int late_load;
};
void launch_deskew_imu_gated(const DeskewPlan& p, const DeskewGate& gate, hipStream_t s);
void launch_deskew_cv(const DeskewPlan& p, const CvArgH& a, hipStream_t s);
struct CvFuseH {
  double rot[9], bias_g[3], vel[3];
  double dt;
  double cov_gyr_scale[3], cov_acc_scale[3];
  const double* st_in;
  double* st_out;
  double* prop_out;
  double* host_out;
  int ctrl_from;
};
void launch_deskew_cv_prop(const DeskewPlan& p, const CvFuseH& f, hipStream_t s);
void launch_deskew_imu_dev(const DeskewPlan& p, const double* pose24_dev, const int* n_poses_dev, const double* poses_dev, hipStream_t s);
constexpr int kImuCarryDoubles = 16;
struct ImuPropArgs {
  const double* st_in;
  const double* samples;
  int n_imu;
  double noise[19];
  double pcl_beg_time, pcl_end_time;
  const float4* scan;
  int n_scan, sorted;
  const unsigned long long* extent;
  const double* carry_in;
  double* carry_out;
  double* poses;
  int* n_poses;
  double* st_out;
  double* prop_out;
  double* host_out;
  const uint4* ctrl_src;
  uint4* ctrl_dst;
  int ctrl_from, ctrl_vec;
};
struct CvPropArgs {
  const double* st_in;
  double dt;
  double cov_gyr_scale[3], cov_acc_scale[3];
  double* st_out;
  double* host_out;
};
void launch_imu_propagate(const ImuPropArgs& a, hipStream_t s);
void launch_cv_propagate(const CvPropArgs& a, hipStream_t s);
void launch_calib_eval(int stage, const double* imu, const double* lidar, int n, const double* params, double* out,
                       hipStream_t s);

void launch_map_decide_compact(const RegistrationBuffers& rb, const PoseArg& ps, double fsd, int have_search, unsigned long long* blk_counts, unsigned int epoch,
                               float4* world, float4* dst_add, float4* dst_nodown, int* counts, int bound_add, int bound_nodown, hipStream_t s,
                               const IekfCtrl* guard = nullptr, int seq = 0, int test_late = 0,
                               unsigned long long* hkey = nullptr, unsigned long long* hbest = nullptr, unsigned int* slot_of = nullptr, float ds = 0.f,
                               unsigned int* ins_flag = nullptr, int* events = nullptr);
void launch_map_publish(const int* ctr, int n_words, int* host, int seq_at, int seq, hipStream_t s);
// ... 103 lines not shown
```

### lidar_imu_init_amd/csrc/lii_scan.hip

```cpp
#include <hip/hip_runtime.h>
#include <string.h>
#include <cstring>
#include <math.h>
#include <stdint.h>

#include "lii_device.h"
#include "lii_imu_dev.h"
#include "lii_launch.h"

namespace lii {

__global__ __launch_bounds__(256) void k_time_extent(const float4* __restrict__ pts, int n, unsigned long long* __restrict__ extent,
                                                     unsigned long long* __restrict__ extent_next, float4* __restrict__ copy_to,
                                                     const uint4* __restrict__ ctrl_src, uint4* __restrict__ ctrl_dst, int ctrl_vec) {
  __shared__ unsigned long long smn[4], smx[4];
  const int n_scan_blocks = gridDim.x - (ctrl_vec > 0 ? 1 : 0);
  if ((int)blockIdx.x == n_scan_blocks) {
    for (int i0 = threadIdx.x; i0 < ctrl_vec; i0 += 256 * 4) {
      uint4 v[4];
#pragma unroll
      for (int u = 0; u < 4; u++) v[u] = i0 + 256 * u < ctrl_vec ? ctrl_src[i0 + 256 * u] : make_uint4(0, 0, 0, 0);
#pragma unroll
      for (int u = 0; u < 4; u++)
        if (i0 + 256 * u < ctrl_vec) ctrl_dst[i0 + 256 * u] = v[u];
    }
    return;
  }
  if (blockIdx.x == 0 && threadIdx.x == 0) { extent_next[0] = ~0ull; extent_next[1] = 0ull; }
  unsigned long long mn = ~0ull, mx = 0;
  const int stride = n_scan_blocks * blockDim.x;
  for (int i = blockIdx.x * blockDim.x + threadIdx.x; i < n; i += 2 * stride) {
    const int i1 = i + stride;
    const float4 p0 = pts[i];
    const float4 p1 = pts[i1 < n ? i1 : i];
    if (copy_to) {
      copy_to[i] = p0;
      if (i1 < n) copy_to[i1] = p1;
    }
    const unsigned int o0 = f2ord(p0.w), o1 = f2ord(p1.w);
    const unsigned long long a0 = ((unsigned long long)o0 << 32) | (unsigned)i;
    const unsigned long long a1 = i1 < n ? (((unsigned long long)o1 << 32) | (unsigned)i1) : ~0ull;
    mn = a0 < mn ? a0 : mn;
    mn = a1 < mn ? a1 : mn;
    mx = (unsigned long long)o0 > mx ? (unsigned long long)o0 : mx;
    mx = (i1 < n && (unsigned long long)o1 > mx) ? (unsigned long long)o1 : mx;
  }
  for (int off = 32; off > 0; off >>= 1) {
    unsigned long long a = __shfl_xor(mn, off), b = __shfl_xor(mx, off);
    mn = a < mn ? a : mn;
    mx = b > mx ? b : mx;
  }
  if ((threadIdx.x & 63) == 0) { smn[threadIdx.x >> 6] = mn; smx[threadIdx.x >> 6] = mx; }
  __syncthreads();
  if (threadIdx.x == 0) {
    for (int w = 1; w < 4; w++) { mn = smn[w] < mn ? smn[w] : mn; mx = smx[w] > mx ? smx[w] : mx; }
    atomicMin(&extent[0], mn);
    atomicMax(&extent[1], mx);
  }
}
__global__ __launch_bounds__(256) void k_sort_keys(const float4* __restrict__ pts, int n, unsigned int* __restrict__ key, unsigned int* __restrict__ idx) {
  const int i = blockIdx.x * blockDim.x + threadIdx.x;
  if (i >= n) return;
  unsigned int u = __float_as_uint(pts[i].w);
  if ((u << 1) == 0u) u = 0u;
  key[i] = f2ord(__uint_as_float(u));
  idx[i] = (unsigned int)i;
}
template <bool INT>
__global__ __launch_bounds__(256) void k_sort_gather(const float4* __restrict__ src, const unsigned int* __restrict__ idx, int n, float4* __restrict__ dst,
                                                     const float* __restrict__ inten_src, float* __restrict__ inten_dst) {
  const int i = blockIdx.x * blockDim.x + threadIdx.x;
  if (i >= n) return;
  const unsigned int j = idx[i];
  if (j < (unsigned int)n) {
    dst[i] = src[j];
    if (INT) inten_dst[i] = inten_src[j];
  }
}
struct UndistArg {
  double endR[9], endp[3], RLI[9], TLI[3];
};

__device__ __forceinline__ void backprop_once(const double* __restrict__ head , double t, const UndistArg& u,
                                              double p[3]) {
  double dt = t - head[0];
  const double* acc = head + 1;
  const double* gyr = head + 4;
  const double* vel = head + 7;
  const double* pos = head + 10;
  const double* rot = head + 13;
  double E[9], Ri[9];
  exp_so3(gyr, dt, E);
  mat3_mul(rot, E, Ri);
  double Pi[3];
#pragma unroll
  for (int a = 0; a < 3; a++) Pi[a] = pos[a] + vel[a] * dt + 0.5 * acc[a] * dt * dt;
  double q[3], w[3], e[3], o[3];
  mat3_vec(u.RLI, p, q);
#pragma unroll
  for (int a = 0; a < 3; a++) q[a] += u.TLI[a];
  mat3_vec(Ri, q, w);
#pragma unroll
  for (int a = 0; a < 3; a++) w[a] = w[a] + Pi[a] - u.endp[a];
  mat3t_vec(u.endR, w, e);
#pragma unroll
  for (int a = 0; a < 3; a++) e[a] -= u.TLI[a];
  mat3t_vec(u.RLI, e, o);
  p[0] = o[0]; p[1] = o[1]; p[2] = o[2];
}

__device__ __forceinline__ void block_bbox_reduce(unsigned int (&lo)[3], unsigned int (&hi)[3]) {
  __shared__ unsigned int s_lo[4][3], s_hi[4][3];
#pragma unroll
  for (int a = 0; a < 3; a++) {
    for (int off = 32; off > 0; off >>= 1) {
      unsigned int x = __shfl_xor(lo[a], off), y = __shfl_xor(hi[a], off);
      lo[a] = min(lo[a], x);
      hi[a] = max(hi[a], y);
    }
  }
  const int wave = threadIdx.x >> 6;
  if ((threadIdx.x & 63) == 0) {
#pragma unroll
    for (int a = 0; a < 3; a++) { s_lo[wave][a] = lo[a]; s_hi[wave][a] = hi[a]; }
  }
  __syncthreads();
  if (threadIdx.x < 3) {
    const int a = threadIdx.x;
    lo[0] = min(min(s_lo[0][a], s_lo[1][a]), min(s_lo[2][a], s_lo[3][a]));
    hi[0] = max(max(s_hi[0][a], s_hi[1][a]), max(s_hi[2][a], s_hi[3][a]));
  }
}
__device__ __forceinline__ void bbox_point(float x, float y, float z, unsigned int (&lo)[3], unsigned int (&hi)[3]) {
  if (isfinite(x) && isfinite(y) && isfinite(z)) {
    const unsigned int ox = f2ord(x), oy = f2ord(y), oz = f2ord(z);
    lo[0] = min(lo[0], ox); hi[0] = max(hi[0], ox);
    lo[1] = min(lo[1], oy); hi[1] = max(hi[1], oy);
    lo[2] = min(lo[2], oz); hi[2] = max(hi[2], oz);
  }
}
__device__ __forceinline__ void deskew_bbox(float4 q, bool in_range, unsigned int* __restrict__ rows, int row) {
  if (!rows) return;
  unsigned int lo[3] = {0xFFFFFFFFu, 0xFFFFFFFFu, 0xFFFFFFFFu}, hi[3] = {0, 0, 0};
  if (in_range) bbox_point(q.x, q.y, q.z, lo, hi);
  block_bbox_reduce(lo, hi);
  if (threadIdx.x < 3) {
    rows[row * 8 + threadIdx.x] = lo[0];
    rows[row * 8 + 4 + threadIdx.x] = hi[0];
  }
}
__device__ __forceinline__ void deskew_bbox(float4 q, bool in_range, unsigned int* __restrict__ rows) { deskew_bbox(q, in_range, rows, (int)blockIdx.x); }

constexpr unsigned int kVhEmpty = 0xFFFFFFFFu;
constexpr int kVhMembers = 10;
struct __attribute__((aligned(64))) VhSlot {
  unsigned long long key;
  unsigned int first;
  unsigned int creator;
  unsigned int count;
  unsigned int head;
  unsigned int members[kVhMembers - 1];
  unsigned int pad;
};
static_assert(sizeof(VhSlot) == 64, "one cache line per slot");
struct VhTable {
  VhSlot* slots;
  unsigned int mask;
  unsigned int* slot_of;
  unsigned int* next;
  unsigned int* crowded;
  unsigned int part_world, part_rank;
  int part_bound;
  int* part_overflow;
};
__device__ __forceinline__ unsigned long long vh_mix(unsigned long long hk) {
  hk ^= hk >> 33; hk *= 0xFF51AFD7ED558CCDull; hk ^= hk >> 33;
  return hk;
}
__device__ __forceinline__ unsigned int voxel_rank(unsigned long long key, unsigned int world) {
  return (unsigned int)(((vh_mix(key) >> 32) * (unsigned long long)world) >> 32);
}
__device__ __forceinline__ void vh_insert(const VhTable& tb, unsigned long long key, int i) {
  unsigned int slot = (unsigned int)vh_mix(key) & tb.mask;
  bool created;
  for (;;) {
    const unsigned long long prev = atomicCAS(&tb.slots[slot].key, ~0ull, key);
    created = prev == ~0ull;
    if (created || prev == key) break;
    slot = (slot + 1u) & tb.mask;
  }
  VhSlot* s = tb.slots + slot;
  if (created) {
    s->creator = (unsigned)i;
  } else {
    atomicMin(&s->first, (unsigned)i);
    const unsigned int k = atomicAdd(&s->count, 1u) + 1u;
    if (k < (unsigned)kVhMembers) s->members[k - 1u] = (unsigned)i;
    else {
      tb.next[i] = atomicExch(&s->head, (unsigned)i);
      if (tb.part_world <= 1u) atomicMax(tb.crowded, k + 1u - (unsigned)kVhMembers);
    }
  }
  tb.slot_of[i] = slot;
}
__device__ __forceinline__ void vhash_insert_abs(const float4 P, int i, float leaf, const VhTable& tb) {
  if (isfinite(P.x) && isfinite(P.y) && isfinite(P.z)) {
    const float inv_leaf = 1.0f / leaf;
    const float fx = floorf(P.x * inv_leaf), fy = floorf(P.y * inv_leaf), fz = floorf(P.z * inv_leaf);
    unsigned long long key;
    if (fabsf(fx) < 1048000.f && fabsf(fy) < 1048000.f && fabsf(fz) < 1048000.f) {
      key = ((unsigned long long)(unsigned)((int)fz + (1 << 20)) << 42) | ((unsigned long long)(unsigned)((int)fy + (1 << 20)) << 21) |
            (unsigned long long)(unsigned)((int)fx + (1 << 20));
    } else {
      key = (1ull << 63) | (unsigned long long)(unsigned)i;
    }
    if (tb.part_world > 1u && voxel_rank(key, tb.part_world) != tb.part_rank) {
      tb.slot_of[i] = kVhEmpty;
      return;
    }
    vh_insert(tb, key, i);
    return;
  }
  tb.slot_of[i] = kVhEmpty;
}

struct DeskewIo {
  const float4* in;
  float4* out;
  int n;
  int sorted;
  const unsigned long long* extent;
  unsigned int* bbox_rows;
  float leaf;
  VhTable tb;
  const uint4* ctrl_src;
  uint4* ctrl_dst;
  int ctrl_vec;
#ifdef LII_GAP_TRACE
  unsigned long long* gap;
#endif
};
__device__ __forceinline__ void gap_trace(const DeskewIo& io) {
#ifdef LII_GAP_TRACE
  if (blockIdx.x == 0 && threadIdx.x == 0 && io.gap) {
    const unsigned long long now = wall_clock64(), prev = io.gap[200];
    if (prev != 0ull && now > prev) {
      if (now - prev < 5000ull) { io.gap[201] += now - prev; io.gap[202] += 1ull; }
      else io.gap[203] += 1ull;
    }
    io.gap[200] = 0ull;
  }
#endif
}
__device__ __forceinline__ void pull_ctrl(const DeskewIo& io) {
  for (int i0 = threadIdx.x; i0 < io.ctrl_vec; i0 += 256 * 4) {
    uint4 v[4];
#pragma unroll
// ... 162 lines not shown
      mat3_vec(R, p, o);
#pragma unroll
      for (int c = 0; c < 3; c++) o[c] = o[c] + (-rv[c]) * dt_j;
      P = make_float4((float)o[0], (float)o[1], (float)o[2], P.w);
      io.out[i] = P;
    } else if (io.in != io.out) {
      io.out[i] = P;
    }
  }
  deskew_bbox(P, in_range, io.bbox_rows);
  if (FUSE && in_range) vhash_insert_abs(P, i, io.leaf, io.tb);
}
template <bool FUSE>
__global__ __launch_bounds__(256) void k_deskew_cv(DeskewIo io, CvArg a) {
  const int n_scan_blocks = gridDim.x - (io.ctrl_vec > 0 ? 1 : 0);
  if ((int)blockIdx.x == n_scan_blocks) { pull_ctrl(io); return; }
  double rv[3];
  mat3t_vec(a.endR, a.vel, rv);
  deskew_cv_point<FUSE>(io, a.omega, rv);
}

struct CvFuseArg {
  double rot[9], bias_g[3], vel[3];
  double dt;
  double cov_gyr_scale[3], cov_acc_scale[3];
  const double* st_in;
  double* st_out;
  double* prop_out;
  double* host_out;
  int ctrl_from;
};
__device__ __forceinline__ void cv_extra_workgroup(const DeskewIo& io, const CvFuseArg& f) {
  __shared__ CvPropLds L;
  const int tid = threadIdx.x;
  const double x = tid < 36 ? f.st_in[tid] : 0.0;
  const double p0 = f.st_in[36 + tid], p1 = f.st_in[36 + 256 + tid], p2 = tid < 64 ? f.st_in[36 + 512 + tid] : 0.0;
  if (io.ctrl_vec > f.ctrl_from) pull_words(io.ctrl_src, io.ctrl_dst, f.ctrl_from, io.ctrl_vec, tid, 256);
  if (tid < 36) L.x[tid] = x;
  L.P[tid] = p0;
  L.P[256 + tid] = p1;
  if (tid < 64) L.P[512 + tid] = p2;
  __syncthreads();
  cv_propagate_lds(L, f.dt, f.cov_gyr_scale, f.cov_acc_scale);
  if (tid < 36) {
    f.st_out[tid] = L.x[tid];
    f.prop_out[tid] = L.x[tid];
    if (f.host_out) f.host_out[tid] = L.x[tid];
  }
  for (int e = tid; e < 576; e += 256) {
    f.st_out[36 + e] = L.P[e];
    if (f.host_out) f.host_out[36 + e] = L.P[e];
  }
}
template <bool FUSE>
__global__ __launch_bounds__(256) void k_deskew_cv_prop(DeskewIo io, CvFuseArg f) {
  if ((int)blockIdx.x == (int)gridDim.x - 1) { cv_extra_workgroup(io, f); return; }
  double endR[9], rv[3];
  cv_end_rotation(f.rot, f.bias_g, f.dt, endR);
  mat3t_vec(endR, f.vel, rv);
#pragma unroll
  for (int c = 0; c < 3; c++) {
    const long long b = __double_as_longlong(rv[c]);
    const unsigned int lo = __builtin_amdgcn_readfirstlane((unsigned int)b), hi = __builtin_amdgcn_readfirstlane((unsigned int)(b >> 32));
    rv[c] = __longlong_as_double((long long)(((unsigned long long)hi << 32) | lo));
  }
  deskew_cv_point<FUSE>(io, f.bias_g, rv);
}

__global__ __launch_bounds__(256) void k_voxel_minmax(const float4* __restrict__ pts, int n, unsigned int* __restrict__ mm,
                                                      unsigned int* __restrict__ mm_next) {
  if (blockIdx.x == 0 && threadIdx.x < 6) mm_next[threadIdx.x] = threadIdx.x < 3 ? 0xFFFFFFFFu : 0u;
  unsigned int lo[3] = {0xFFFFFFFFu, 0xFFFFFFFFu, 0xFFFFFFFFu}, hi[3] = {0, 0, 0};
  for (int i = blockIdx.x * blockDim.x + threadIdx.x; i < n; i += gridDim.x * blockDim.x) {
    const float4 p = pts[i];
    bbox_point(p.x, p.y, p.z, lo, hi);
  }
  block_bbox_reduce(lo, hi);
  if (threadIdx.x < 3) {
    atomicMin(&mm[threadIdx.x], lo[0]);
    atomicMax(&mm[3 + threadIdx.x], hi[0]);
  }
}

struct VoxelArg {
  float inv_leaf;
  int min_b[3];
  int mul[3];
  int identity;
};
__device__ __forceinline__ VoxelArg voxel_prepare(const unsigned int* __restrict__ mm, float leaf) {
  VoxelArg v;
  v.inv_leaf = 1.0f / leaf;
  v.identity = 0;
  for (int a = 0; a < 3; a++) { v.min_b[a] = 0; v.mul[a] = 0; }
  if (mm[0] != 0xFFFFFFFFu) {
    float mn[3], mx[3];
    for (int a = 0; a < 3; a++) {
      unsigned int lo = mm[a], hi = mm[3 + a];
      unsigned int ul = (lo & 0x80000000u) ? (lo & 0x7FFFFFFFu) : ~lo, uh = (hi & 0x80000000u) ? (hi & 0x7FFFFFFFu) : ~hi;
      mn[a] = __uint_as_float(ul);
      mx[a] = __uint_as_float(uh);
    }
    long long dx = (long long)((mx[0] - mn[0]) * v.inv_leaf) + 1, dy = (long long)((mx[1] - mn[1]) * v.inv_leaf) + 1,
              dz = (long long)((mx[2] - mn[2]) * v.inv_leaf) + 1;
    if (dx * dy * dz > 2147483647LL) {
      v.identity = 1;
    } else {
      int div_b[3];
      for (int a = 0; a < 3; a++) {
        v.min_b[a] = (int)floorf(mn[a] * v.inv_leaf);
        div_b[a] = (int)floorf(mx[a] * v.inv_leaf) - v.min_b[a] + 1;
      }
      v.mul[0] = 1; v.mul[1] = div_b[0]; v.mul[2] = div_b[0] * div_b[1];
    }
  }
  return v;
}
__global__ __launch_bounds__(256) void k_voxel_keys(const float4* __restrict__ pts, int n, const unsigned int* __restrict__ mm,
                                                    const unsigned int* __restrict__ bbox_rows, int n_rows, float leaf,
                                                    unsigned long long* __restrict__ keys, unsigned int* __restrict__ pcl_keys,
                                                    int* __restrict__ filtered,
                                                    unsigned long long* __restrict__ samples, int sample_width) {
  __shared__ unsigned int s_mm[8];
  if (n_rows > 0) {
    unsigned int lo[3] = {0xFFFFFFFFu, 0xFFFFFFFFu, 0xFFFFFFFFu}, hi[3] = {0, 0, 0};
    for (int r = threadIdx.x; r < n_rows; r += 256) {
      const uint4 a = *reinterpret_cast<const uint4*>(bbox_rows + r * 8), b = *reinterpret_cast<const uint4*>(bbox_rows + r * 8 + 4);
      lo[0] = min(lo[0], a.x); lo[1] = min(lo[1], a.y); lo[2] = min(lo[2], a.z);
      hi[0] = max(hi[0], b.x); hi[1] = max(hi[1], b.y); hi[2] = max(hi[2], b.z);
    }
    block_bbox_reduce(lo, hi);
    if (threadIdx.x < 3) { s_mm[threadIdx.x] = lo[0]; s_mm[3 + threadIdx.x] = hi[0]; }
    __syncthreads();
    mm = s_mm;
  }
  int i = blockIdx.x * blockDim.x + threadIdx.x;
  if (i >= n) return;
  const VoxelArg v = voxel_prepare(mm, leaf);
  if (i == 0) *filtered = v.identity ? 0 : 1;
  float4 p = pts[i];
  unsigned long long key = kVoxDropKey;
  unsigned int pcl = 0x7FFFFFFFu;
  if (v.identity) {
    key = pcl = (unsigned)i;
  } else if (isfinite(p.x) && isfinite(p.y) && isfinite(p.z)) {
    int i0 = (int)(floorf(p.x * v.inv_leaf) - (float)v.min_b[0]);
    int i1 = (int)(floorf(p.y * v.inv_leaf) - (float)v.min_b[1]);
    int i2 = (int)(floorf(p.z * v.inv_leaf) - (float)v.min_b[2]);
    pcl = (unsigned)(i0 * v.mul[0] + i1 * v.mul[1] + i2 * v.mul[2]);
    key = pcl;
  }
  keys[i] = key;
  pcl_keys[i] = pcl;
  if (samples) {
    const unsigned int j = (unsigned int)i / (unsigned int)sample_width, lo = j * (unsigned int)sample_width;
    unsigned int hsh = j * 2654435761u;
    hsh ^= hsh >> 15; hsh *= 2246822519u; hsh ^= hsh >> 13;
    const unsigned int w = min((unsigned int)sample_width, (unsigned int)n - lo);
    if (lo + hsh % w == (unsigned int)i) samples[j] = (key << kVoxIdxBits) | (unsigned long long)(unsigned int)i;
  }
}
__global__ __launch_bounds__(256) void k_vh_clear(VhSlot* slots, unsigned int n_slots) {
  const unsigned int i = blockIdx.x * blockDim.x + threadIdx.x;
  if (i >= n_slots) return;
  VhSlot s;
  s.key = ~0ull; s.first = kVhEmpty; s.creator = kVhEmpty; s.count = 0u; s.head = kVhEmpty; s.pad = 0u;
#pragma unroll
  for (int k = 0; k < kVhMembers - 1; k++) s.members[k] = kVhEmpty;
  slots[i] = s;
}
__device__ __forceinline__ void fold_bbox_rows(const unsigned int* __restrict__ bbox_rows, int n_rows, unsigned int* s_mm ) {
  unsigned int lo[3] = {0xFFFFFFFFu, 0xFFFFFFFFu, 0xFFFFFFFFu}, hi[3] = {0, 0, 0};
  for (int r = threadIdx.x; r < n_rows; r += 256) {
    const uint4 a = *reinterpret_cast<const uint4*>(bbox_rows + r * 8), b = *reinterpret_cast<const uint4*>(bbox_rows + r * 8 + 4);
    lo[0] = min(lo[0], a.x); lo[1] = min(lo[1], a.y); lo[2] = min(lo[2], a.z);
    hi[0] = max(hi[0], b.x); hi[1] = max(hi[1], b.y); hi[2] = max(hi[2], b.z);
  }
  block_bbox_reduce(lo, hi);
  if (threadIdx.x < 3) { s_mm[threadIdx.x] = lo[0]; s_mm[3 + threadIdx.x] = hi[0]; }
  __syncthreads();
}
__global__ __launch_bounds__(256) void k_vhash_insert(const float4* __restrict__ pts, int n, const unsigned int* __restrict__ mm,
                                                      const unsigned int* __restrict__ bbox_rows, int n_rows, float leaf,
                                                      VhTable tb, int* __restrict__ filtered) {
  __shared__ unsigned int s_mm[8];
  if (n_rows > 0) {
    fold_bbox_rows(bbox_rows, n_rows, s_mm);
    mm = s_mm;
  }
  const int i = blockIdx.x * blockDim.x + threadIdx.x;
  if (i >= n) return;
  const VoxelArg v = voxel_prepare(mm, leaf);
  if (i == 0) *filtered = v.identity ? 0 : 1;
  const float4 p = pts[i];
  unsigned long long key = ~0ull;
  if (v.identity) {
    key = (unsigned)i;
  } else if (isfinite(p.x) && isfinite(p.y) && isfinite(p.z)) {
    const int i0 = (int)(floorf(p.x * v.inv_leaf) - (float)v.min_b[0]);
    const int i1 = (int)(floorf(p.y * v.inv_leaf) - (float)v.min_b[1]);
    const int i2 = (int)(floorf(p.z * v.inv_leaf) - (float)v.min_b[2]);
    key = (unsigned)(i0 * v.mul[0] + i1 * v.mul[1] + i2 * v.mul[2]);
  }
  if (key != ~0ull) vh_insert(tb, key, i);
  else tb.slot_of[i] = kVhEmpty;
}
__device__ __forceinline__ unsigned int block_rank_of_flag(bool f, unsigned int* s_w , unsigned int* total) {
  const unsigned long long b = __ballot(f);
  const int lane = threadIdx.x & 63, wave = threadIdx.x >> 6;
  if (lane == 0) s_w[wave] = (unsigned)__popcll(b);
  __syncthreads();
  unsigned int before = 0;
  for (int w = 0; w < wave; w++) before += s_w[w];
  *total = s_w[0] + s_w[1] + s_w[2] + s_w[3];
  return before + (unsigned)__popcll(b & ((1ull << lane) - 1ull));
}
template <bool ABS, bool INT>
__global__ __launch_bounds__(256) void k_vhash_emit(const float4* __restrict__ pts, int n, VhTable tb, unsigned long long* __restrict__ counts,
                                                    unsigned int epoch, float4* __restrict__ out, int* __restrict__ n_out,
                                                    unsigned int* __restrict__ pcl_out, const unsigned int* __restrict__ bbox_rows,
                                                    int n_rows, float leaf, int* __restrict__ filtered, int test_late,
                                                    const float* __restrict__ inten, float* __restrict__ inten_out) {
  __shared__ unsigned int s_w[4], s_sum[12];
  const int tid = threadIdx.x, i = blockIdx.x * blockDim.x + tid;
  const bool in_range = i < n;
  const float4 p0 = in_range ? pts[i] : make_float4(0.f, 0.f, 0.f, 0.f);
  const unsigned int slot = in_range ? tb.slot_of[i] : kVhEmpty;
  const float q0 = (INT && in_range) ? inten[i] : 0.f;
  VoxelArg v;
  v.identity = 0;
  if (ABS) {
    __shared__ unsigned int s_mm[8];
    fold_bbox_rows(bbox_rows, n_rows, s_mm);
    v = voxel_prepare(s_mm, leaf);
    if (i == 0) *filtered = v.identity ? 0 : 1;
  }
  VhSlot* const sl = tb.slots + (slot != kVhEmpty ? slot : 0u);
  uint4 hd = make_uint4(0u, 0u, kVhEmpty, 0u), m0 = make_uint4(kVhEmpty, kVhEmpty, kVhEmpty, kVhEmpty), m1 = m0;
  uint2 m2 = make_uint2(kVhEmpty, kVhEmpty);
  unsigned long long key = 0;
  if (slot != kVhEmpty) {
    const uint4* line = reinterpret_cast<const uint4*>(sl);
    const uint4 a = line[0];
    key = ((unsigned long long)a.y << 32) | a.x;
    hd.x = a.z;
    m0.x = a.w;
    const uint4 b = line[1];
    hd.y = b.x; hd.z = b.y;
    m0.y = b.z; m0.z = b.w;
    const uint4 c = line[2], d = line[3];
    m0.w = c.x; m1 = make_uint4(c.y, c.z, c.w, d.x); m2 = make_uint2(d.y, d.z);
  }
  const bool ident_part = ABS && v.identity && tb.part_world > 1u;
  const bool first = slot != kVhEmpty && (ident_part || min(hd.x, m0.x) == (unsigned)i);
  unsigned int total;
  const unsigned int rank = block_rank_of_flag(first, s_w, &total);
  const bool hold = test_late != 0 && (blockIdx.x % 7u) == 3u && !(ABS && v.identity && !ident_part);
  if (tid == 0 && !hold) __hip_atomic_store(counts + blockIdx.x, ((unsigned long long)epoch << 32) | total, __ATOMIC_RELAXED, __HIP_MEMORY_SCOPE_AGENT);
  if (ABS && v.identity && !ident_part) {
    if (in_range) { out[i] = p0; pcl_out[i] = (unsigned)i; }
    if (INT && in_range) inten_out[i] = q0;
    if (blockIdx.x == gridDim.x - 1 && tid == 0) *n_out = n;
    if (first) {
      uint4* line = reinterpret_cast<uint4*>(sl);
      line[0] = make_uint4(0xFFFFFFFFu, 0xFFFFFFFFu, kVhEmpty, kVhEmpty);
      line[1] = make_uint4(0u, kVhEmpty, kVhEmpty, kVhEmpty);
    }
    return;
  }
  float4 cen = make_float4(0.f, 0.f, 0.f, 0.f);
  float cen_i = 0.f;
  if (first) {
    const unsigned int cnt = ident_part ? 1u : hd.y + 1u;
    float sx = __fadd_rn(0.f, p0.x), sy = __fadd_rn(0.f, p0.y), sz = __fadd_rn(0.f, p0.z), st = __fadd_rn(0.f, p0.w);
    float si = INT ? __fadd_rn(0.f, q0) : 0.f;
    unsigned int m[kVhMembers] = {m0.x, m0.y, m0.z, m0.w, m1.x, m1.y, m1.z, m1.w, m2.x, m2.y};
#pragma unroll
    for (int k = 0; k < kVhMembers; k++)
      if ((unsigned)k >= cnt) m[k] = kVhEmpty;
    if (cnt > 512u) {
#pragma unroll
      for (int k = 0; k < kVhMembers; k++) {
        if (m[k] == (unsigned)i || m[k] == kVhEmpty) continue;
        const float4 p = pts[m[k]];
        sx = __fadd_rn(sx, p.x); sy = __fadd_rn(sy, p.y); sz = __fadd_rn(sz, p.z); st = __fadd_rn(st, p.w);
        if (INT) si = __fadd_rn(si, inten[m[k]]);
      }
      for (unsigned int j = hd.z; j != kVhEmpty; j = tb.next[j]) {
        if (j == (unsigned)i) continue;
        const float4 p = pts[j];
        sx = __fadd_rn(sx, p.x); sy = __fadd_rn(sy, p.y); sz = __fadd_rn(sz, p.z); st = __fadd_rn(st, p.w);
        if (INT) si = __fadd_rn(si, inten[j]);
      }
    } else if (cnt > 1u) {
      const unsigned int head = cnt > (unsigned)kVhMembers ? hd.z : kVhEmpty;
      unsigned int last = (unsigned)i;
      for (unsigned int r = 1; r < cnt; r++) {
        unsigned int best = kVhEmpty;
// ... 216 lines not shown
```

Measured before the change: 7748 scans/s.

## Fuse voxel-hash emit stage into the first KNN search kernel

The voxel-hash emit launch after downsampling is now deferred and recorded as a plan. The first KNN pass of the iterated EKF update then runs a new fused kernel that computes voxel centroids, places them through a decoupled look-back prefix over 64-point blocks, and starts the neighbor search in the same launch. This removes a kernel launch and a global round trip of downsampled points between emit and the first search. The cost is a more complex kernel that carries extra shared memory and atomic prefix logic, which may lower occupancy. Fallback flushes keep any other path that needs the emit output correct.

```diff
diff --git a/lidar_imu_init_amd/csrc/lii_capi.cpp b/lidar_imu_init_amd/csrc/lii_capi.cpp
--- a/lidar_imu_init_amd/csrc/lii_capi.cpp
+++ b/lidar_imu_init_amd/csrc/lii_capi.cpp
@@ -86,8 +86,18 @@
   if (h->vh.part_world > 1) return true;
   return h->vh_mode == 1 && (h->vh_pinned || leaf == h->vh_leaf);
 }
+int emit_flush(lii_handle h) {
+  if (!h->emit_pending) return LII_OK;
+  h->emit_pending = false;
+  const EmitKnnPlan& ep = h->emit_plan;
+  launch_voxel_hash(*ep.vh, ep.pts, ep.n, nullptr, ep.bbox_rows, ep.n_rows, ep.leaf, ep.out, ep.n_out, ep.filtered, ep.pcl_out, 4, ep.vh_epoch, h->stream, ep.test_late,
+                    ep.inten, ep.inten_out);
+  HIPCHK(h, hipGetLastError());
+  return LII_OK;
+}
 int resolve_n_body(lii_handle h) {
   if (!h->n_body_pending) return LII_OK;
+  { const int rce = emit_flush(h); if (rce != LII_OK) return rce; }
   HIPCHK(h, hipMemcpyAsync(h->h_small + 2048, h->d_nbody, 2 * sizeof(int), hipMemcpyDeviceToHost, h->stream));
   HIPCHK(h, hipStreamSynchronize(h->stream));
   int v[2];
@@ -228,6 +238,7 @@
   if (const char* v = std::getenv("LII_MAP_FUSE")) h->map_fuse = v[0] != '0';
   if (const char* v = std::getenv("LII_WIDE_COMPLETION")) h->wide_enabled = v[0] != '0';
   if (const char* v = std::getenv("LII_INGEST_SORT")) h->ingest_sort_always = v[0] == 'a';
+  if (const char* v = std::getenv("LII_FUSED_FIRST_SEARCH")) h->fused_first_search = v[0] != '0';
   if (const char* v = std::getenv("LII_PREARM")) h->pre.enabled = std::atoi(v) != 0;
   if (const char* v = std::getenv("LII_PREARM_TIMEOUT_MS")) h->pre.timeout_ticks = std::max(1ll, (long long)(std::atof(v) * 1e5));
   if (const char* v = std::getenv("LII_MAILBOX_TIMEOUT_S")) {
@@ -331,6 +342,7 @@
   if (std::string(prop.gcnArchName).find("gfx950") == std::string::npos)
     return fail(h, LII_ERR_NO_DEVICE, std::string("device is ") + prop.gcnArchName + ", kernels are built for gfx950 only");
   HIPCHK(h, h->stream.create(hipStreamNonBlocking));
+  h->fused_max_points = 64 * 7 * std::max(prop.multiProcessorCount, 1);
   const size_t N = size_t(cfg->max_scan_points), M = size_t(cfg->max_map_points);
   const size_t NM = std::max(N, M);
   HIPCHK(h, h->d_map_unsorted.alloc(M));
@@ -455,7 +467,7 @@
     h->vh.slots = h->vh_slots;
     launch_voxel_hash_clear(h->vh, slots, h->stream);
     HIPCHK(h, h->vh_slot_of.alloc(N)); HIPCHK(h, h->vh_next.alloc(N));
-    HIPCHK(h, h->vh_counts.alloc(N / 256 + 8)); HIPCHK(h, hipMemset(h->vh_counts, 0, 8 * (N / 256 + 8)));
+    HIPCHK(h, h->vh_counts.alloc(N / 64 + 16)); HIPCHK(h, hipMemset(h->vh_counts, 0, 8 * (N / 64 + 16)));
     HIPCHK(h, h->vh_crowded.alloc(4));
     HIPCHK(h, hipMemset(h->vh_crowded, 0, 16));
     h->vh.slot_of = h->vh_slot_of; h->vh.next = h->vh_next; h->vh.counts = h->vh_counts; h->vh.crowded = h->vh_crowded;
@@ -800,7 +812,10 @@
     return LII_OK;
   }
   hipStream_t s = h->stream;
-  if (h->prof.kp_active) { const int r = kp_mark(h, LII_KP_VOXEL); if (r != LII_OK) return r; }
+  const bool defer = h->emit_defer && h->vh_inserted && leaf == h->vh_inserted_leaf && h->bbox_rows > 0 && h->vh.part_world <= 1 && !n_down && !filtered &&
+                     n <= h->fused_max_points;
+  h->emit_defer = false;
+  if (h->prof.kp_active && !defer) { const int r = kp_mark(h, LII_KP_VOXEL); if (r != LII_OK) return r; }
   unsigned int* mm = h->d_mm + 8 * h->mm_sel;
   if (h->bbox_rows == 0) {
     h->mm_sel ^= 1;
@@ -836,7 +851,15 @@
   const bool by_voxel = inserted && h->vh.part_world > 1;
   if (use_hash) {
     if (++h->vh_epoch == 0u) h->vh_epoch = 1u;
-    launch_voxel_hash(h->vh, h->d_scan, n, mm, h->d_bbox_rows, h->bbox_rows, leaf, h->d_body, h->d_nbody, h->d_nbody + 1, h->d_vpcl_out, hash_stages, h->vh_epoch, s, h->test_emit_late ? 1 : 0, inten, inten_out);
+    if (defer) {
+      EmitKnnPlan& ep = h->emit_plan;
+      ep.vh = &h->vh; ep.pts = h->d_scan; ep.n = n; ep.bbox_rows = h->d_bbox_rows; ep.n_rows = h->bbox_rows; ep.leaf = leaf;
+      ep.out = h->d_body; ep.n_out = h->d_nbody; ep.filtered = h->d_nbody + 1; ep.pcl_out = h->d_vpcl_out;
+      ep.vh_epoch = h->vh_epoch; ep.test_late = h->test_emit_late ? 1 : 0; ep.inten = inten; ep.inten_out = inten_out;
+      h->emit_pending = true;
+    } else {
+      launch_voxel_hash(h->vh, h->d_scan, n, mm, h->d_bbox_rows, h->bbox_rows, leaf, h->d_body, h->d_nbody, h->d_nbody + 1, h->d_vpcl_out, hash_stages, h->vh_epoch, s, h->test_emit_late ? 1 : 0, inten, inten_out);
+    }
     if (!h->vh_pinned && !by_voxel && !h->vh_flag_pending && (++h->vh_watch & 15) == 0) {
       HIPCHK(h, hipMemcpyAsync(h->h_vh_crowded, h->vh.crowded, sizeof(unsigned int), hipMemcpyDeviceToHost, s));
       HIPCHK(h, hipMemsetAsync(h->vh.crowded, 0, sizeof(unsigned int), s));
diff --git a/lidar_imu_init_amd/csrc/lii_capi_register.cpp b/lidar_imu_init_amd/csrc/lii_capi_register.cpp
--- a/lidar_imu_init_amd/csrc/lii_capi_register.cpp
+++ b/lidar_imu_init_amd/csrc/lii_capi_register.cpp
@@ -15,6 +15,11 @@
 void launch_knn(lii_handle h, const GridView& g, const RegistrationBuffers& rb, const PoseArg* pose, int forced, int epoch,
                 hipEvent_t ev_start = nullptr, hipEvent_t ev_stop = nullptr) {
   lii::launch_knn(g, rb, pose, h->d_ctrl, forced, h->d_ctrl->search_pose, h->stream, epoch, ev_start, ev_stop);
+}
+void launch_emit_knn(lii_handle h, const GridView& g, const RegistrationBuffers& rb, const PoseArg* pose, int forced, int epoch,
+                     hipEvent_t ev_start = nullptr, hipEvent_t ev_stop = nullptr) {
+  h->emit_pending = false;
+  lii::launch_emit_knn(h->emit_plan, g, rb, pose, h->d_ctrl, forced, h->d_ctrl->search_pose, h->stream, epoch, ev_start, ev_stop);
 }
 
 
@@ -118,7 +123,13 @@
   auto enqueue_pass = [&](int it) -> int {
     const bool knn = it >= 16 || ((plan >> it) & 1u);
     const int epoch = knn ? next_knn_epoch(h) : 0;
-    if (knn) {
+    const bool with_emit = h->emit_pending && knn && it == 0;
+    if (h->emit_pending && !with_emit) { const int r = emit_flush(h); if (r != LII_OK) return r; }
+    if (knn && with_emit) {
+      if (h->prof.kp_active) { const int r = kp_mark(h, LII_KP_KNN, it); if (r != LII_OK) return r; }
+      if (prof) launch_emit_knn(h, g, rb, pose, -1, epoch, h->prof.ev_it[0], h->prof.ev_it[1]);
+      else launch_emit_knn(h, g, rb, pose, -1, epoch);
+    } else if (knn) {
       if (h->prof.kp_active) { const int r = kp_mark(h, LII_KP_KNN, it); if (r != LII_OK) return r; }
       if (prof && it < 16) launch_knn(h, g, rb, pose, -1, epoch, h->prof.ev_it[2 * it], h->prof.ev_it[2 * it + 1]);
       else launch_knn(h, g, rb, pose, -1, epoch);
@@ -615,7 +626,10 @@
     HIPCHK(h, hipMemcpyAsync(h->d_ctrl, h->h_ctrl, h->ctrl_pending, hipMemcpyHostToDevice, h->stream));
     h->ctrl_pending = 0;
   }
+  h->emit_defer = rc == LII_OK && job->leaf > 0 && h->fused_first_search && !h->host_solve && !h->net.comm && h->net.n_ranks <= 1 && h->solo_share == 0 &&
+                  !h->wide_listed && h->prof.prof_mode != 3;
   if (rc == LII_OK) rc = job->leaf > 0 ? lii_downsample(h, job->leaf, nullptr, nullptr) : lii_downsample_skip(h, nullptr);
+  h->emit_defer = false;
   const auto t_pre = std::chrono::steady_clock::now();
   const bool map_update = job->struct_size >= 56u && job->map_update == 1;
   h->map_after_update = map_update && !h->host_solve;
@@ -624,6 +638,10 @@
   h->wait_hook_arg = job->struct_size >= 88u ? job->while_waiting_arg : nullptr;
   h->lm.in_job = local_map && rc == LII_OK;
   if (rc == LII_OK) rc = lii_iekf_update(h, state, state_prop ? state_prop : state, &job->opts, report);
+  if (h->emit_pending) {
+    const int rce = emit_flush(h);
+    if (rc == LII_OK) rc = rce;
+  }
   if (h->lm.in_job) {
     if (rc == LII_OK) local_map_settle(h);
     else h->lm.counts_pending = true;
diff --git a/lidar_imu_init_amd/csrc/lii_context.h b/lidar_imu_init_amd/csrc/lii_context.h
--- a/lidar_imu_init_amd/csrc/lii_context.h
+++ b/lidar_imu_init_amd/csrc/lii_context.h
@@ -178,6 +178,10 @@
   float fuse_leaf = 0.f;
   float vh_inserted_leaf = 0.f;
   bool vh_inserted = false;
+  bool fused_first_search = true;
+  bool emit_defer = false, emit_pending = false;
+  int fused_max_points = 0;
+  lii::EmitKnnPlan emit_plan = {};
   int vh_mode = 1;
   float vh_leaf = -1.f;
   unsigned int vh_watch = 0;
@@ -359,6 +363,7 @@
 PoseArg pose_of(const lii_state& s);
 int resolve_n_body(lii_handle h);
 bool fuse_filter(lii_handle h, float leaf);
+int emit_flush(lii_handle h);
 int pcl_order(lii_handle h, const int** perm);
 void extent_discard(lii_handle h);
 int scan_sort_into(lii_handle h, const float4* src, int n);
diff --git a/lidar_imu_init_amd/csrc/lii_knn.hip b/lidar_imu_init_amd/csrc/lii_knn.hip
--- a/lidar_imu_init_amd/csrc/lii_knn.hip
+++ b/lidar_imu_init_amd/csrc/lii_knn.hip
@@ -2,9 +2,12 @@
 #include <hip/hip_ext.h>
 #include <math.h>
 #include <stdint.h>
+#include <string.h>
+#include <type_traits>
 #include <utility>
 
 #include "lii_search.h"
+#include "lii_voxel.h"
 #include "lii_launch.h"
 
 namespace lii {
@@ -209,15 +212,258 @@
     }
   }
 }
-template <int LPQ, int BS, int NB, int WPE>
-__global__ __launch_bounds__(BS, WPE) void k_knn_ck(GridView g, RegistrationBuffers rb, const PoseArg* __restrict__ pose,
+struct EmitKnnArg {
+  const float4* pts;
+  int n;
+  VhTable tb;
+  unsigned long long* counts;
+  unsigned int epoch;
+  float4* out;
+  int* n_out;
+  int* filtered;
+  unsigned int* pcl_out;
+  const unsigned int* bbox_rows;
+  int n_rows;
+  float leaf;
+  int test_late;
+  const float* inten;
+  float* inten_out;
+};
+struct NoEmit {};
+constexpr int kEkPts = 64;
+struct EmitShared {
+  float4 cen[kEkPts];
+  unsigned int pcl[kEkPts];
+  float inten[kEkPts];
+  unsigned int slot[kEkPts];
+  unsigned int w[4], sum[12], mm[8], look[8];
+};
+template <bool EMIT>
+__device__ __forceinline__ EmitShared* emit_shared() {
+  if constexpr (EMIT) {
+    __shared__ EmitShared s;
+    return &s;
+  } else {
+    return nullptr;
+  }
+}
+struct EmitState {
+  unsigned int total;
+  bool ident;
+  bool hold;
+};
+template <bool INT>
+__device__ __forceinline__ EmitState emit_phase(const EmitKnnArg& ea, EmitShared* __restrict__ es, const int blk, const float4 p0, const unsigned int slot,
+                                                const float q0) {
+  const int tid = threadIdx.x, i = blk * kEkPts + tid;
+  const bool in_range = tid < kEkPts && i < ea.n;
+  fold_bbox_rows(ea.bbox_rows, ea.n_rows, es->mm);
+  const VoxelArg v = voxel_prepare(es->mm, ea.leaf);
+  EmitState st;
+  st.ident = __builtin_amdgcn_readfirstlane(v.identity) != 0;
+  const bool ident = st.ident;
+  if (blk == 0 && tid == 0) *ea.filtered = ident ? 0 : 1;
+  uint4 la = make_uint4(0u, 0u, kVhEmpty, kVhEmpty), lb = make_uint4(0u, kVhEmpty, kVhEmpty, kVhEmpty),
+        lc = make_uint4(kVhEmpty, kVhEmpty, kVhEmpty, kVhEmpty), ld = lc;
+  if (slot != kVhEmpty) {
+    const uint4* line = reinterpret_cast<const uint4*>(ea.tb.slots + slot);
+    la = line[0]; lb = line[1]; lc = line[2]; ld = line[3];
+  }
+  const bool first = slot != kVhEmpty && min(la.z, la.w) == (unsigned)i;
+  const bool leaves = ident ? in_range : first;
+  const unsigned int rank = block_rank_of_flag(leaves, es->w, &st.total);
+  st.hold = ea.test_late != 0 && ((unsigned)blk % 7u) == 3u && !ident;
+  if (tid == 0 && !st.hold && !ident)
+    __hip_atomic_store(ea.counts + blk, ((unsigned long long)ea.epoch << 32) | st.total, __ATOMIC_RELAXED, __HIP_MEMORY_SCOPE_AGENT);
+  if (tid < kEkPts) {
+    float4 cen = p0;
+    float cen_i = q0;
+    unsigned int pcl = (unsigned)i;
+    if (first && !ident) {
+      const unsigned int cnt = lb.x + 1u;
+      float sx = __fadd_rn(0.f, p0.x), sy = __fadd_rn(0.f, p0.y), sz = __fadd_rn(0.f, p0.z), st_ = __fadd_rn(0.f, p0.w);
+      float si = INT ? __fadd_rn(0.f, q0) : 0.f;
+      unsigned int m[kVhMembers] = {la.w, lb.z, lb.w, lc.x, lc.y, lc.z, lc.w, ld.x, ld.y, ld.z};
+#pragma unroll
+      for (int k = 0; k < kVhMembers; k++)
+        if ((unsigned)k >= cnt) m[k] = kVhEmpty;
+      const unsigned int last_pt = (unsigned)ea.n - 1u;
+      auto add = [&](unsigned int j) {
+        const float4 p = ea.pts[j];
+        sx = __fadd_rn(sx, p.x); sy = __fadd_rn(sy, p.y); sz = __fadd_rn(sz, p.z); st_ = __fadd_rn(st_, p.w);
+        if (INT) si = __fadd_rn(si, ea.inten[j]);
+      };
+      if (cnt > 512u) {
+#pragma unroll
+        for (int k = 0; k < kVhMembers; k++)
+          if (m[k] != (unsigned)i && m[k] != kVhEmpty) add(m[k]);
+        for (unsigned int j = lb.y; j != kVhEmpty; j = ea.tb.next[j])
+          if (j != (unsigned)i) add(j);
+      } else if (cnt > (unsigned)kVhMembers) {
+        unsigned int last = (unsigned)i;
+        for (unsigned int r = 1; r < cnt; r++) {
+          unsigned int best = kVhEmpty;
+#pragma unroll
+          for (int k = 0; k < kVhMembers; k++) best = (m[k] > last && m[k] < best) ? m[k] : best;
+          for (unsigned int j = lb.y; j != kVhEmpty; j = ea.tb.next[j]) best = (j > last && j < best) ? j : best;
+          add(min(best, last_pt));
+          last = best;
+        }
+      } else if (cnt > 1u) {
+#pragma unroll
+        for (int k = 0; k < kVhMembers; k++) m[k] = m[k] == (unsigned)i ? kVhEmpty : m[k];
+#pragma unroll
+        for (int pass = 0; pass < kVhMembers; pass++)
+#pragma unroll
+          for (int k = pass & 1; k + 1 < kVhMembers; k += 2) {
+            const unsigned int a = min(m[k], m[k + 1]), b = max(m[k], m[k + 1]);
+            m[k] = a; m[k + 1] = b;
+          }
+        const unsigned int nm = cnt - 1u;
+#pragma unroll
+        for (int b0 = 0; b0 < kVhMembers - 1; b0 += 4) {
+          if (nm > (unsigned)b0) {
+            float4 P[4];
+            float Q[4];
+#pragma unroll
+            for (int u = 0; u < 4; u++) {
+              if (b0 + u < kVhMembers - 1) {
+                const unsigned int j = min(m[b0 + u], last_pt);
+                P[u] = ea.pts[j];
+                Q[u] = INT ? ea.inten[j] : 0.f;
+              }
+            }
+#pragma unroll
+            for (int u = 0; u < 4; u++) {
+              if (b0 + u < kVhMembers - 1 && (unsigned)(b0 + u) < nm) {
+                sx = __fadd_rn(sx, P[u].x); sy = __fadd_rn(sy, P[u].y); sz = __fadd_rn(sz, P[u].z); st_ = __fadd_rn(st_, P[u].w);
+                if (INT) si = __fadd_rn(si, Q[u]);
+              }
+            }
+          }
+        }
+      }
+      const float c = (float)cnt;
+      cen = make_float4(sx / c, sy / c, sz / c, st_ / c);
+      if (INT) cen_i = si / c;
+      pcl = voxel_pcl_index(v, p0.x, p0.y, p0.z);
+    }
+    if (leaves) {
+      es->cen[rank] = cen;
+      es->pcl[rank] = pcl;
+      if (INT) es->inten[rank] = cen_i;
+    }
+    es->slot[tid] = first ? slot : kVhEmpty;
+  }
+  __syncthreads();
+  return st;
+}
+template <bool INT>
+__device__ __forceinline__ int emit_place(const EmitKnnArg& ea, EmitShared* __restrict__ es, const EmitState& st, const int blk, const int nb_real) {
+  const int tid = threadIdx.x;
+  __builtin_amdgcn_s_waitcnt(0x0F70);
+  unsigned int base = (unsigned)blk * (unsigned)kEkPts;
+  if (!st.ident) {
+    unsigned int seen = 0;
+    bool missing = false;
+    for (int q0 = tid; q0 < blk; q0 += 256 * 8) {
+      unsigned long long v[8];
+#pragma unroll
+      for (int u = 0; u < 8; u++)
+        v[u] = q0 + 256 * u < blk ? __hip_atomic_load(ea.counts + q0 + 256 * u, __ATOMIC_RELAXED, __HIP_MEMORY_SCOPE_AGENT) : ((unsigned long long)ea.epoch << 32);
+#pragma unroll
+      for (int u = 0; u < 8; u++) {
+        missing = missing || (unsigned int)(v[u] >> 32) != ea.epoch;
+        seen += (unsigned int)v[u] & 0xFFFFu;
+      }
+    }
+#pragma unroll
+    for (int off = 32; off > 0; off >>= 1) seen += __shfl_down(seen, off);
+    const bool wave_missing = __any(missing);
+    if ((tid & 63) == 0) { es->look[tid >> 6] = seen; es->look[4 + (tid >> 6)] = wave_missing ? 1u : 0u; }
+    __syncthreads();
+    if (__builtin_amdgcn_readfirstlane(es->look[4] | es->look[5] | es->look[6] | es->look[7]) == 0u) {
+      base = es->look[0] + es->look[1] + es->look[2] + es->look[3];
+    } else
+    base = prefix_below(ea.counts, ea.epoch, blk, es->sum, ea.test_late != 0, [&](int q) -> unsigned int {
+      const int j = q * kEkPts + tid;
+      bool f = false;
+      if (tid < kEkPts && j < ea.n) {
+        const unsigned int sq = ea.tb.slot_of[j];
+        if (sq != kVhEmpty) {
+          const uint4 a = *reinterpret_cast<const uint4*>(ea.tb.slots + sq);
+          f = min(a.z, a.w) == (unsigned)j;
+        }
+      }
+      unsigned int tot;
+      (void)block_rank_of_flag(f, es->w, &tot);
+      return tot;
+    }).y;
+  }
+  if (st.hold) {
+    if (tid == 0) {
+      __hip_atomic_store(ea.counts + blk, ((unsigned long long)ea.epoch << 32) | st.total, __ATOMIC_RELAXED, __HIP_MEMORY_SCOPE_AGENT);
+      __builtin_amdgcn_s_waitcnt(0x0F70);
+    }
+    __syncthreads();
+  }
+  if (blk == nb_real - 1 && tid == 0) *ea.n_out = st.ident ? ea.n : (int)(base + st.total);
+  if (tid < (int)st.total) {
+    const unsigned int pos = base + (unsigned)tid;
+    ea.out[pos] = es->cen[tid];
+    ea.pcl_out[pos] = es->pcl[tid];
+    if (INT) ea.inten_out[pos] = es->inten[tid];
+  }
+  return (int)base;
+}
+__device__ __forceinline__ void emit_free(const EmitKnnArg& ea, const EmitShared* __restrict__ es) {
+  if (threadIdx.x < kEkPts) {
+    const unsigned int so = es->slot[threadIdx.x];
+    if (so != kVhEmpty) {
+      uint4* line = reinterpret_cast<uint4*>(ea.tb.slots + so);
+      line[0] = make_uint4(0xFFFFFFFFu, 0xFFFFFFFFu, kVhEmpty, kVhEmpty);
+      line[1] = make_uint4(0u, kVhEmpty, kVhEmpty, kVhEmpty);
+    }
+  }
+}
+
+template <int LPQ, int BS, int NB, int WPE, class EA, bool INT>
+__global__ __launch_bounds__(BS, WPE) void k_knn_ck(GridView g, RegistrationBuffers rb, EA ea, const PoseArg* __restrict__ pose,
                                                const IekfCtrl* __restrict__ ctrl, int forced, int nb_real,
                                                double* __restrict__ search_pose_out, int epoch) {
   using G = CkGeom<LPQ>;
+  constexpr bool kEmit = std::is_same<EA, EmitKnnArg>::value;
   constexpr int QPB = BS / LPQ;
+  static_assert(!kEmit || (LPQ == 4 && QPB == kEkPts), "the emit phase: 64 input points and up to 64 queries per workgroup");
   __shared__ unsigned int s_tab[QPB * (G::MAXCH + NB)];
   const int blk = xcd_remap(blockIdx.x, nb_real);
   const int sub = threadIdx.x & (LPQ - 1);
+  int qi = 0;
+  bool live = false;
+  float wx = 0, wy = 0, wz = 0;
+  EmitState em = {};
+  if constexpr (kEmit) {
+    const int tid = threadIdx.x, i = blk * kEkPts + tid;
+    const bool in_range = tid < kEkPts && i < ea.n;
+    const float4 p0 = in_range ? ea.pts[i] : make_float4(0.f, 0.f, 0.f, 0.f);
+    const unsigned int slot = in_range ? ea.tb.slot_of[i] : kVhEmpty;
+    const float q0 = (INT && in_range) ? ea.inten[i] : 0.f;
+    const HeadScalars hs = load_head_scalars(pose, &ctrl->search_next, &ctrl->max_it, &ctrl->max_it);
+    if (epoch > 0 && blockIdx.x == 0 && tid == 0) rb.flag_count[(epoch + 1) & 1] = 0;
+    const bool due = !(forced < 0 && (hs.stop || !hs.search_next));
+    if (due && search_pose_out && blockIdx.x == 0 && tid < 24) search_pose_out[tid] = pose_element(hs.ps, tid);
+    if (blk >= nb_real) return;
+    EmitShared* const es = emit_shared<kEmit>();
+    em = emit_phase<INT>(ea, es, blk, p0, slot, q0);
+    const int r = tid / LPQ;
+    live = r < (int)em.total;
+    if (!due || __builtin_amdgcn_readfirstlane((tid & ~63) / LPQ) >= __builtin_amdgcn_readfirstlane((int)em.total)) {
+      (void)emit_place<INT>(ea, es, em, blk, nb_real);
+      emit_free(ea, es);
+      return;
+    }
+    if (live && sub == 0) body_to_world(hs.ps, es->cen[r], wx, wy, wz);
+  } else {
   const int ql = blk * QPB + (int)(threadIdx.x / LPQ);
   const bool early = rb.shard_world <= 1;
   float4 pb_early = make_float4(0.f, 0.f, 0.f, 0.f);
@@ -232,10 +478,10 @@
   if (search_pose_out && blockIdx.x == 0 && threadIdx.x < 24) search_pose_out[threadIdx.x] = pose_element(ps, threadIdx.x);
   if (blk >= nb_real) return;
   if (blk * QPB + (int)((threadIdx.x & ~63u) / LPQ) >= n_live) return;
-  const int qi = lo + ql;
-  const bool live = ql < n_live;
-  float wx = 0, wy = 0, wz = 0;
+  qi = lo + ql;
+  live = ql < n_live;
   if (live && sub == 0) body_to_world(ps, early ? pb_early : rb.body[qi], wx, wy, wz);
+  }
   wx = group_bcast_f<LPQ, 0>(wx); wy = group_bcast_f<LPQ, 0>(wy); wz = group_bcast_f<LPQ, 0>(wz);
   const bool active = live && g.n_pts > 0;
   const float INF = __builtin_inff();
@@ -407,6 +653,7 @@
   const int found = e[4] < INF ? 5 : (e[3] < INF ? 4 : (e[2] < INF ? 3 : (e[1] < INF ? 2 : (e[0] < INF ? 1 : 0))));
   const bool amb = d7t < INF && !(d5 < d7t);
   const bool need = active && (ovf || amb || !(fminf(d5, g.max_d2) <= guardsq));
+  if constexpr (kEmit) qi = emit_place<INT>(ea, emit_shared<kEmit>(), em, blk, nb_real) + (int)(threadIdx.x / LPQ);
   if (live) {
     static_for<G::NW>([&](auto ic) {
       constexpr int i = decltype(ic)::value;
@@ -432,6 +679,7 @@
     }
     if (sub == (LPQ == 4 ? 2 : 0)) rb.world[qi] = make_float4(wx, wy, wz, 0.f);
   }
+  if constexpr (kEmit) emit_free(ea, emit_shared<kEmit>());
 }
 
 static inline int nblk(int n, int b) { return (n + b - 1) / b; }
@@ -441,11 +689,41 @@
   int nq = nblk(shard_bound(rb), kKnnBs / 4);
   if (nq < 1) nq = 1;
   const int nq_pad = ((nq + 7) / 8) * 8;
+  const NoEmit ne;
   if (ev_start && ev_stop) {
-    hipExtLaunchKernelGGL((k_knn_ck<4, kKnnBs, kKnnNb, kKnnWpe>), dim3(nq_pad), dim3(kKnnBs), 0, s, ev_start, ev_stop, 0u, g, rb, pose, ctrl, forced, nq,
-                          search_pose_out, epoch);
+    hipExtLaunchKernelGGL((k_knn_ck<4, kKnnBs, kKnnNb, kKnnWpe, NoEmit, false>), dim3(nq_pad), dim3(kKnnBs), 0, s, ev_start, ev_stop, 0u, g, rb, ne, pose, ctrl,
+                          forced, nq, search_pose_out, epoch);
     return;
   }
-  hipLaunchKernelGGL((k_knn_ck<4, kKnnBs, kKnnNb, kKnnWpe>), dim3(nq_pad), dim3(kKnnBs), 0, s, g, rb, pose, ctrl, forced, nq, search_pose_out, epoch);
-}
-}
+  hipLaunchKernelGGL((k_knn_ck<4, kKnnBs, kKnnNb, kKnnWpe, NoEmit, false>), dim3(nq_pad), dim3(kKnnBs), 0, s, g, rb, ne, pose, ctrl, forced, nq, search_pose_out, epoch);
+}
+template <bool INT>
+static void launch_emit_knn_t(int nb, const GridView& g, const RegistrationBuffers& rb, const EmitKnnArg& ea, const PoseArg* pose, const IekfCtrl* ctrl,
+                              int forced, double* search_pose_out, hipStream_t s, int epoch, hipEvent_t ev_start, hipEvent_t ev_stop) {
+  const int nb_pad = ((nb + 7) / 8) * 8;
+  constexpr int BS = 4 * kEkPts;
+  if (ev_start && ev_stop) {
+    hipExtLaunchKernelGGL((k_knn_ck<4, BS, kKnnNb, kKnnWpe, EmitKnnArg, INT>), dim3(nb_pad), dim3(BS), 0, s, ev_start, ev_stop, 0u, g, rb, ea, pose, ctrl, forced,
+                          nb, search_pose_out, epoch);
+    return;
+  }
+  hipLaunchKernelGGL((k_knn_ck<4, BS, kKnnNb, kKnnWpe, EmitKnnArg, INT>), dim3(nb_pad), dim3(BS), 0, s, g, rb, ea, pose, ctrl, forced, nb, search_pose_out, epoch);
+}
+void launch_emit_knn(const EmitKnnPlan& p, const GridView& g, const RegistrationBuffers& rb, const PoseArg* pose, const IekfCtrl* ctrl, int forced,
+                     double* search_pose_out, hipStream_t s, int epoch, hipEvent_t ev_start, hipEvent_t ev_stop) {
+  if (p.n <= 0) return;
+  EmitKnnArg ea;
+  memset(&ea, 0, sizeof(ea));
+  ea.pts = p.pts; ea.n = p.n;
+  ea.tb.slots = static_cast<VhSlot*>(p.vh->slots);
+  ea.tb.mask = (unsigned int)voxel_hash_slots(p.n) - 1u;
+  ea.tb.slot_of = p.vh->slot_of; ea.tb.next = p.vh->next; ea.tb.crowded = p.vh->crowded;
+  ea.counts = p.vh->counts; ea.epoch = p.vh_epoch;
+  ea.out = p.out; ea.n_out = p.n_out; ea.filtered = p.filtered; ea.pcl_out = p.pcl_out;
+  ea.bbox_rows = p.bbox_rows; ea.n_rows = p.n_rows; ea.leaf = p.leaf; ea.test_late = p.test_late;
+  ea.inten = p.inten; ea.inten_out = p.inten_out;
+  const int nb = nblk(p.n, kEkPts);
+  if (p.inten && p.inten_out) launch_emit_knn_t<true>(nb, g, rb, ea, pose, ctrl, forced, search_pose_out, s, epoch, ev_start, ev_stop);
+  else launch_emit_knn_t<false>(nb, g, rb, ea, pose, ctrl, forced, search_pose_out, s, epoch, ev_start, ev_stop);
+}
+}
diff --git a/lidar_imu_init_amd/csrc/lii_launch.h b/lidar_imu_init_amd/csrc/lii_launch.h
--- a/lidar_imu_init_amd/csrc/lii_launch.h
+++ b/lidar_imu_init_amd/csrc/lii_launch.h
@@ -104,6 +104,24 @@
                        int n_rows, float leaf, float4* out, int* n_out, int* filtered, unsigned int* pcl_out, int stages, unsigned int epoch,
                        hipStream_t s, int test_late = 0 ,
                        const float* inten = nullptr, float* inten_out = nullptr);
+struct EmitKnnPlan {
+  const VoxelHashBuffers* vh;
+  const float4* pts;
+  int n;
+  const unsigned int* bbox_rows;
+  int n_rows;
+  float leaf;
+  float4* out;
+  int* n_out;
+  int* filtered;
+  unsigned int* pcl_out;
+  unsigned int vh_epoch;
+  int test_late;
+  const float* inten;
+  float* inten_out;
+};
+void launch_emit_knn(const EmitKnnPlan& p, const GridView& g, const RegistrationBuffers& rb, const PoseArg* pose, const IekfCtrl* ctrl, int forced,
+                     double* search_pose_out, hipStream_t s, int epoch, hipEvent_t ev_start = nullptr, hipEvent_t ev_stop = nullptr);
 struct DeskewPlan {
   const float4* in;
   float4* out;
diff --git a/lidar_imu_init_amd/csrc/lii_scan.hip b/lidar_imu_init_amd/csrc/lii_scan.hip
--- a/lidar_imu_init_amd/csrc/lii_scan.hip
+++ b/lidar_imu_init_amd/csrc/lii_scan.hip
@@ -6,6 +6,7 @@
 
 #include "lii_device.h"
 #include "lii_imu_dev.h"
+#include "lii_voxel.h"
 #include "lii_launch.h"
 
 namespace lii {
@@ -109,28 +110,6 @@
   p[0] = o[0]; p[1] = o[1]; p[2] = o[2];
 }
 
-__device__ __forceinline__ void block_bbox_reduce(unsigned int (&lo)[3], unsigned int (&hi)[3]) {
-  __shared__ unsigned int s_lo[4][3], s_hi[4][3];
-#pragma unroll
-  for (int a = 0; a < 3; a++) {
-    for (int off = 32; off > 0; off >>= 1) {
-      unsigned int x = __shfl_xor(lo[a], off), y = __shfl_xor(hi[a], off);
-      lo[a] = min(lo[a], x);
-      hi[a] = max(hi[a], y);
-    }
-  }
-  const int wave = threadIdx.x >> 6;
-  if ((threadIdx.x & 63) == 0) {
-#pragma unroll
-    for (int a = 0; a < 3; a++) { s_lo[wave][a] = lo[a]; s_hi[wave][a] = hi[a]; }
-  }
-  __syncthreads();
-  if (threadIdx.x < 3) {
-    const int a = threadIdx.x;
-    lo[0] = min(min(s_lo[0][a], s_lo[1][a]), min(s_lo[2][a], s_lo[3][a]));
-    hi[0] = max(max(s_hi[0][a], s_hi[1][a]), max(s_hi[2][a], s_hi[3][a]));
-  }
-}
 __device__ __forceinline__ void bbox_point(float x, float y, float z, unsigned int (&lo)[3], unsigned int (&hi)[3]) {
   if (isfinite(x) && isfinite(y) && isfinite(z)) {
     const unsigned int ox = f2ord(x), oy = f2ord(y), oz = f2ord(z);
@@ -151,28 +130,6 @@
 }
 __device__ __forceinline__ void deskew_bbox(float4 q, bool in_range, unsigned int* __restrict__ rows) { deskew_bbox(q, in_range, rows, (int)blockIdx.x); }
 
-constexpr unsigned int kVhEmpty = 0xFFFFFFFFu;
-constexpr int kVhMembers = 10;
-struct __attribute__((aligned(64))) VhSlot {
-  unsigned long long key;
-  unsigned int first;
-  unsigned int creator;
-  unsigned int count;
-  unsigned int head;
-  unsigned int members[kVhMembers - 1];
-  unsigned int pad;
-};
-static_assert(sizeof(VhSlot) == 64, "one cache line per slot");
-struct VhTable {
-  VhSlot* slots;
-  unsigned int mask;
-  unsigned int* slot_of;
-  unsigned int* next;
-  unsigned int* crowded;
-  unsigned int part_world, part_rank;
-  int part_bound;
-  int* part_overflow;
-};
 __device__ __forceinline__ unsigned long long vh_mix(unsigned long long hk) {
   hk ^= hk >> 33; hk *= 0xFF51AFD7ED558CCDull; hk ^= hk >> 33;
   return hk;
@@ -501,40 +458,6 @@
   }
 }
 
-struct VoxelArg {
-  float inv_leaf;
-  int min_b[3];
-  int mul[3];
-  int identity;
-};
-__device__ __forceinline__ VoxelArg voxel_prepare(const unsigned int* __restrict__ mm, float leaf) {
-  VoxelArg v;
-  v.inv_leaf = 1.0f / leaf;
-  v.identity = 0;
-  for (int a = 0; a < 3; a++) { v.min_b[a] = 0; v.mul[a] = 0; }
-  if (mm[0] != 0xFFFFFFFFu) {
-    float mn[3], mx[3];
-    for (int a = 0; a < 3; a++) {
-      unsigned int lo = mm[a], hi = mm[3 + a];
-      unsigned int ul = (lo & 0x80000000u) ? (lo & 0x7FFFFFFFu) : ~lo, uh = (hi & 0x80000000u) ? (hi & 0x7FFFFFFFu) : ~hi;
-      mn[a] = __uint_as_float(ul);
-      mx[a] = __uint_as_float(uh);
-    }
-    long long dx = (long long)((mx[0] - mn[0]) * v.inv_leaf) + 1, dy = (long long)((mx[1] - mn[1]) * v.inv_leaf) + 1,
-              dz = (long long)((mx[2] - mn[2]) * v.inv_leaf) + 1;
-    if (dx * dy * dz > 2147483647LL) {
-      v.identity = 1;
-    } else {
-      int div_b[3];
-      for (int a = 0; a < 3; a++) {
-        v.min_b[a] = (int)floorf(mn[a] * v.inv_leaf);
-        div_b[a] = (int)floorf(mx[a] * v.inv_leaf) - v.min_b[a] + 1;
-      }
-      v.mul[0] = 1; v.mul[1] = div_b[0]; v.mul[2] = div_b[0] * div_b[1];
-    }
-  }
-  return v;
-}
 __global__ __launch_bounds__(256) void k_voxel_keys(const float4* __restrict__ pts, int n, const unsigned int* __restrict__ mm,
                                                     const unsigned int* __restrict__ bbox_rows, int n_rows, float leaf,
                                                     unsigned long long* __restrict__ keys, unsigned int* __restrict__ pcl_keys,
@@ -588,17 +511,6 @@
   for (int k = 0; k < kVhMembers - 1; k++) s.members[k] = kVhEmpty;
   slots[i] = s;
 }
-__device__ __forceinline__ void fold_bbox_rows(const unsigned int* __restrict__ bbox_rows, int n_rows, unsigned int* s_mm ) {
-  unsigned int lo[3] = {0xFFFFFFFFu, 0xFFFFFFFFu, 0xFFFFFFFFu}, hi[3] = {0, 0, 0};
-  for (int r = threadIdx.x; r < n_rows; r += 256) {
-    const uint4 a = *reinterpret_cast<const uint4*>(bbox_rows + r * 8), b = *reinterpret_cast<const uint4*>(bbox_rows + r * 8 + 4);
-    lo[0] = min(lo[0], a.x); lo[1] = min(lo[1], a.y); lo[2] = min(lo[2], a.z);
-    hi[0] = max(hi[0], b.x); hi[1] = max(hi[1], b.y); hi[2] = max(hi[2], b.z);
-  }
-  block_bbox_reduce(lo, hi);
-  if (threadIdx.x < 3) { s_mm[threadIdx.x] = lo[0]; s_mm[3 + threadIdx.x] = hi[0]; }
-  __syncthreads();
-}
 __global__ __launch_bounds__(256) void k_vhash_insert(const float4* __restrict__ pts, int n, const unsigned int* __restrict__ mm,
                                                       const unsigned int* __restrict__ bbox_rows, int n_rows, float leaf,
                                                       VhTable tb, int* __restrict__ filtered) {
@@ -623,16 +535,6 @@
   }
   if (key != ~0ull) vh_insert(tb, key, i);
   else tb.slot_of[i] = kVhEmpty;
-}
-__device__ __forceinline__ unsigned int block_rank_of_flag(bool f, unsigned int* s_w , unsigned int* total) {
-  const unsigned long long b = __ballot(f);
-  const int lane = threadIdx.x & 63, wave = threadIdx.x >> 6;
-  if (lane == 0) s_w[wave] = (unsigned)__popcll(b);
-  __syncthreads();
-  unsigned int before = 0;
-  for (int w = 0; w < wave; w++) before += s_w[w];
-  *total = s_w[0] + s_w[1] + s_w[2] + s_w[3];
-  return before + (unsigned)__popcll(b & ((1ull << lane) - 1ull));
 }
 template <bool ABS, bool INT>
 __global__ __launch_bounds__(256) void k_vhash_emit(const float4* __restrict__ pts, int n, VhTable tb, unsigned long long* __restrict__ counts,
diff --git a/lidar_imu_init_amd/csrc/lii_voxel.h b/lidar_imu_init_amd/csrc/lii_voxel.h
--- /dev/null
+++ b/lidar_imu_init_amd/csrc/lii_voxel.h
@@ -0,0 +1,114 @@
+#pragma once
+#include "lii_device.h"
+
+namespace lii {
+
+__device__ __forceinline__ void block_bbox_reduce(unsigned int (&lo)[3], unsigned int (&hi)[3]) {
+  __shared__ unsigned int s_lo[4][3], s_hi[4][3];
+#pragma unroll
+  for (int a = 0; a < 3; a++) {
+    for (int off = 32; off > 0; off >>= 1) {
+      unsigned int x = __shfl_xor(lo[a], off), y = __shfl_xor(hi[a], off);
+      lo[a] = min(lo[a], x);
+      hi[a] = max(hi[a], y);
+    }
+  }
+  const int wave = threadIdx.x >> 6;
+  if ((threadIdx.x & 63) == 0) {
+#pragma unroll
+    for (int a = 0; a < 3; a++) { s_lo[wave][a] = lo[a]; s_hi[wave][a] = hi[a]; }
+  }
+  __syncthreads();
+  if (threadIdx.x < 3) {
+    const int a = threadIdx.x;
+    lo[0] = min(min(s_lo[0][a], s_lo[1][a]), min(s_lo[2][a], s_lo[3][a]));
+    hi[0] = max(max(s_hi[0][a], s_hi[1][a]), max(s_hi[2][a], s_hi[3][a]));
+  }
+}
+
+constexpr unsigned int kVhEmpty = 0xFFFFFFFFu;
+constexpr int kVhMembers = 10;
+struct __attribute__((aligned(64))) VhSlot {
+  unsigned long long key;
+  unsigned int first;
+  unsigned int creator;
+  unsigned int count;
+  unsigned int head;
+  unsigned int members[kVhMembers - 1];
+  unsigned int pad;
+};
+static_assert(sizeof(VhSlot) == 64, "one cache line per slot");
+struct VhTable {
+  VhSlot* slots;
+  unsigned int mask;
+  unsigned int* slot_of;
+  unsigned int* next;
+  unsigned int* crowded;
+  unsigned int part_world, part_rank;
+  int part_bound;
+  int* part_overflow;
+};
+
+struct VoxelArg {
+  float inv_leaf;
+  int min_b[3];
+  int mul[3];
+  int identity;
+};
+__device__ __forceinline__ VoxelArg voxel_prepare(const unsigned int* __restrict__ mm, float leaf) {
+  VoxelArg v;
+  v.inv_leaf = 1.0f / leaf;
+  v.identity = 0;
+  for (int a = 0; a < 3; a++) { v.min_b[a] = 0; v.mul[a] = 0; }
+  if (mm[0] != 0xFFFFFFFFu) {
+    float mn[3], mx[3];
+    for (int a = 0; a < 3; a++) {
+      unsigned int lo = mm[a], hi = mm[3 + a];
+      unsigned int ul = (lo & 0x80000000u) ? (lo & 0x7FFFFFFFu) : ~lo, uh = (hi & 0x80000000u) ? (hi & 0x7FFFFFFFu) : ~hi;
+      mn[a] = __uint_as_float(ul);
+      mx[a] = __uint_as_float(uh);
+    }
+    long long dx = (long long)((mx[0] - mn[0]) * v.inv_leaf) + 1, dy = (long long)((mx[1] - mn[1]) * v.inv_leaf) + 1,
+              dz = (long long)((mx[2] - mn[2]) * v.inv_leaf) + 1;
+    if (dx * dy * dz > 2147483647LL) {
+      v.identity = 1;
+    } else {
+      int div_b[3];
+      for (int a = 0; a < 3; a++) {
+        v.min_b[a] = (int)floorf(mn[a] * v.inv_leaf);
+        div_b[a] = (int)floorf(mx[a] * v.inv_leaf) - v.min_b[a] + 1;
+      }
+      v.mul[0] = 1; v.mul[1] = div_b[0]; v.mul[2] = div_b[0] * div_b[1];
+    }
+  }
+  return v;
+}
+__device__ __forceinline__ unsigned int voxel_pcl_index(const VoxelArg& v, float x, float y, float z) {
+  const int i0 = (int)(floorf(x * v.inv_leaf) - (float)v.min_b[0]);
+  const int i1 = (int)(floorf(y * v.inv_leaf) - (float)v.min_b[1]);
+  const int i2 = (int)(floorf(z * v.inv_leaf) - (float)v.min_b[2]);
+  return (unsigned)(i0 * v.mul[0] + i1 * v.mul[1] + i2 * v.mul[2]);
+}
+__device__ __forceinline__ void fold_bbox_rows(const unsigned int* __restrict__ bbox_rows, int n_rows, unsigned int* s_mm ) {
+  unsigned int lo[3] = {0xFFFFFFFFu, 0xFFFFFFFFu, 0xFFFFFFFFu}, hi[3] = {0, 0, 0};
+  for (int r = threadIdx.x; r < n_rows; r += 256) {
+    const uint4 a = *reinterpret_cast<const uint4*>(bbox_rows + r * 8), b = *reinterpret_cast<const uint4*>(bbox_rows + r * 8 + 4);
+    lo[0] = min(lo[0], a.x); lo[1] = min(lo[1], a.y); lo[2] = min(lo[2], a.z);
+    hi[0] = max(hi[0], b.x); hi[1] = max(hi[1], b.y); hi[2] = max(hi[2], b.z);
+  }
+  block_bbox_reduce(lo, hi);
+  if (threadIdx.x < 3) { s_mm[threadIdx.x] = lo[0]; s_mm[3 + threadIdx.x] = hi[0]; }
+  __syncthreads();
+}
+__device__ __forceinline__ unsigned int block_rank_of_flag(bool f, unsigned int* s_w , unsigned int* total) {
+  const unsigned long long b = __ballot(f);
+  const int lane = threadIdx.x & 63, wave = threadIdx.x >> 6;
+  if (lane == 0) s_w[wave] = (unsigned)__popcll(b);
+  __syncthreads();
+  unsigned int before = 0;
+  for (int w = 0; w < wave; w++) before += s_w[w];
+  *total = s_w[0] + s_w[1] + s_w[2] + s_w[3];
+  return before + (unsigned)__popcll(b & ((1ull << lane) - 1ull));
+}
+
+}
```

Measured after the change: 7798 scans/s (median of 6 runs). No clear change (+0.6%).
